# nka77/DAHiTra

Measured on AMD Instinct MI355X. Metric: image-pairs/s (256x256) train step, 1/2/4/8 MI355X + CPU ref, higher is better.
Workload: dtype bf16; 1 GPU; LEVIR-CD 256x256 synthetic pairs, base_transformer_pos_s4, bf16, batch 32 per GPU (global 32), fwd+focal+bwd+allreduce+AdamW; net_G=base_transformer_pos_s4, global_batch=32, img_size=256, parallelism=dp1, hip_graph=True, step_form=one graph (AdamW inside), attn_dtype=bf16

## Files before the change

dahitra_amd/csrc/conv_wgrad.hip:

```cpp
#include "common.h"

namespace {

constexpr int TH = 8, TW = 16;
static inline int co_tile(int Cout) { return Cout <= 16 ? 16 : (Cout <= 32 ? 32 : 64); }

struct WgArgs {
    const void* x;
    const void* dy;
    float* part;
    int N, H, W, Cin, OH, OW, Cout, pad;
    int tilesX, tilesY, splitk, groups, npix, in_npix;
    int ci_tiles;
    int CinPitch;
    int dil;
    int CoutUse;
    int direct;
    const float* in_scale;
    const float* in_shift;
    int in_groups;
    int phase_mode;
    int no_xcd_remap;
    const void* dyt_y;
    const float* dytoef;
    int dyt_groups;
    long x_split;
};

constexpr int lds_pitch(int row_bytes) { return ((row_bytes / 32) & 1) ? row_bytes : row_bytes + 32; }

union F8 {
    s16x8 v;
    s16x4 h[2];
// ... 523 lines not shown
    const int t = threadIdx.x;
    if (t < (vec ? 128 : 32)) {
        const int l2 = vec ? t >> 2 : t, e = vec ? t & 3 : 0;
        const long i2 = vec ? (block * 32 + l2) * 4 + e : block * 32 + l2;
        if (i2 < n) {
            float s = 0.f;
#pragma unroll
            for (int r = 0; r < 8; ++r) s += red[r][l2 * 4 + e];
            const int ci2 = (int)(i2 % I), o2 = (int)((i2 / I) % O), tap2 = (int)(i2 / ((long)I * O));
            const size_t d = ((size_t)o2 * I + ci2) * taps + tap2;
            if (accumulate) dw[d] += s; else dw[d] = s;
        }
    }
}
__global__ void wgrad_reduce_oihw_kernel(const float* __restrict__ part, int splitk, int taps, int Oslab, int O, int I,
                                         float* __restrict__ dw, int accumulate) {
    __shared__ float red[8][132];
    const long n = (long)O * I * taps;
    wgrad_reduce_block(part + (size_t)blockIdx.y * splitk * taps * Oslab * I, splitk, taps, Oslab, O, I,
                       dw + (size_t)blockIdx.y * n, accumulate, blockIdx.x, red);
}
struct WgReduceJob {
    const float* part;
    float* dw;
    int splitk, taps, Oslab, O, I, accumulate, first_block, nblocks;
};
__global__ void wgrad_reduce_multi_kernel(const WgReduceJob* __restrict__ jobs, int njobs) {
    __shared__ float red[8][132];
    int j = 0;
    while (j + 1 < njobs && (int)blockIdx.x >= jobs[j + 1].first_block) ++j;
    const WgReduceJob job = jobs[j];
    wgrad_reduce_block(job.part, job.splitk, job.taps, job.Oslab, job.O, job.I, job.dw, job.accumulate,
                       (long)blockIdx.x - job.first_block, red);
}

#ifdef DH_WS_TIMING
__device__ long long g_ws[4096 * 16];
#define WS_NOW() ((long long)wall_clock64())
#define WS_T(...) __VA_ARGS__
#else
#define WS_T(...)
#endif
template <int DIL>
__device__ __forceinline__ void ws_body(const WgArgs& p, int bx, int kz, const int nbx, const int nkz, unsigned char* smem) {
    constexpr int KS = 3, TAPS = 9;
    constexpr int HH = (TH - 1) + (KS - 1) * DIL + 1, HWD = (TW - 1) + (KS - 1) * DIL + 1;
    constexpr int XP = lds_pitch(128), DP = lds_pitch(128);
    constexpr int STAGE = HH * HWD * XP + TH * TW * DP;
    float* bnp = reinterpret_cast<float*>(smem + 2 * STAGE);

    const int tid = threadIdx.x, lane = tid & 63, wv = tid >> 6;
    const int pl = lane & 15, g = lane >> 4;
    if (nbx > 1 && (nkz & 7) == 0 && !p.no_xcd_remap) {
        const unsigned lin = (unsigned)(kz * nbx + bx), xcd = lin & 7, sq = lin >> 3;
        bx = (int)(sq % nbx);
        kz = (int)((sq / nbx) * 8 + xcd);
    }
    const int cot = bx / p.ci_tiles, cit = bx % p.ci_tiles;
    const int co0 = cot * 64, ci0 = cit * 64;
    const int tiles_per_img = p.tilesX * p.tilesY;
    const int ntiles = p.N * tiles_per_img;
    const int my_tiles = kz < ntiles ? (ntiles - kz + p.splitk - 1) / p.splitk : 0;

    if (p.in_scale) {
        for (int i = tid; i < p.in_groups * 128; i += 512) {
            const int gi = i >> 7, k = (i >> 6) & 1, c = i & 63;
// ... 668 lines not shown
                                     int H, int W, int Cin, int OH, int OW, int Cout, int ks, int stride, int pad,
                                     int use_tr, int Cout_real, int dilation, const float* in_scale, const float* in_shift,
                                     int in_groups, void* workspace, int* splitk_out, void* stream) {
    DH_REQUIRE(in_scale && in_shift, "conv2d_wgrad_bn_in: scale / shift missing");
    return conv2d_wgrad_impl(dtype, x, dy, dw_oihw, accumulate, N, H, W, Cin, OH, OW, Cout, ks, stride, pad, 1, 0, use_tr,
                             Cout_real, 0, dilation, workspace, stream, splitk_out ? 1 : 0, splitk_out, in_scale, in_shift,
                             in_groups);
}
extern "C" int dh_conv2d_wgrad_describe(int dtype, int accumulate, int N, int H, int W, int Cin, int OH, int OW, int Cout, int ks,
                                        int stride, int pad, int groups, int npix_valid, int use_tr, int Cout_real, int cin_pitch,
                                        int dilation, int in_groups, int has_in_scale, int split_input, int batch_open, int* out) {
    static const float on[1] = {0.f};
    DH_REQUIRE(out, "conv2d_wgrad_describe: out missing");
    return conv2d_wgrad_impl(dtype, nullptr, nullptr, nullptr, accumulate, N, H, W, Cin, OH, OW, Cout, ks, stride, pad, groups, npix_valid,
                             use_tr, Cout_real, split_input ? Cin / 2 : cin_pitch, dilation, nullptr, nullptr, 1, nullptr,
                             has_in_scale ? on : nullptr, has_in_scale ? on : nullptr, in_groups, nullptr, nullptr, 1,
                             split_input ? 16 : 0, out, batch_open, ks == 2);
}
extern "C" int dh_stem_wgrad_bn(const void* xs16, const void* d, const void* y, const float* coef, int groups, int N, int OH,
                                int OW, float* dw2, int use_tr, void* workspace, void* stream) {
    DH_REQUIRE(xs16 && d && y && coef && groups >= 1 && N % groups == 0, "stem_wgrad_bn: bad arguments (N=%d groups=%d)", N, groups);
    return conv2d_wgrad_impl(DH_DTYPE_BF16, xs16, d, dw2, 0, N, OH, OW, 16, OH, OW, 64, 4, 1, 2, 1, 0, use_tr, 0, 16, 1, workspace,
                             stream, 0, nullptr, nullptr, nullptr, 1, y, coef, groups);
}
extern "C" int dh_wgrad_reduce_job_size(void) { return (int)sizeof(WgReduceJob); }
extern "C" int dh_wgrad_reduce_outputs_per_block(int Cin) { return wgrad_reduce_epb(Cin); }
extern "C" int dh_wgrad_reduce_multi(const void* jobs_dev, int njobs, int total_blocks, void* stream) {
    if (njobs <= 0) return 0;
    hipLaunchKernelGGL(wgrad_reduce_multi_kernel, dim3(total_blocks), dim3(256), 0, reinterpret_cast<hipStream_t>(stream),
                       reinterpret_cast<const WgReduceJob*>(jobs_dev), njobs);
    DH_CHECK_LAUNCH("wgrad_reduce_multi");
    return 0;
}

extern "C" long dh_conv2d_wgrad_phase_workspace_size(int N, int H, int W, int Cin) {
    WgArgs a = wg_args(N, H, W, Cin, H, W, 32, 1);
    a.phase_mode = 1;
    WgPlan p;
    wg_plan(a, WgLaunch{WG_BF16, true, 2, 1, 0, false}, p);
    return (long)4 * p.splitk * 4 * 32 * Cin * 4;
}
extern "C" int dh_conv2d_wgrad_phase(int dtype, const void* x, const void* dy, int N, int H, int W, int Cin, int use_tr,
                                     void* workspace, int* splitk_out, void* stream) {
    DH_REQUIRE(splitk_out && workspace, "conv2d_wgrad_phase: workspace / splitk_out missing");
    DH_REQUIRE((Cin * (dtype == DH_DTYPE_BF16 ? 2 : 4)) % 16 == 0, "conv2d_wgrad_phase: Cin=%d not 16-byte aligned", Cin);
    return conv2d_wgrad_impl(dtype, x, dy, nullptr, 0, N, H, W, Cin, H, W, 32, 2, 1, 1, 1, 0, use_tr, 0, 0, 1, workspace, stream, 1,
                             splitk_out, nullptr, nullptr, 1, nullptr, nullptr, 1, 0, nullptr, 0, 1);
}

namespace {
__global__ void phase_wgrad_combine_kernel(const float* __restrict__ dwab, float* __restrict__ dw, int Cin, int accumulate) {
    const int i = blockIdx.x * blockDim.x + threadIdx.x;
    if (i >= 32 * Cin) return;
    const size_t pstride = (size_t)32 * Cin * 4;
    const float* src = dwab + (size_t)i * 4;
    float v[4][4];
#pragma unroll
    for (int ph = 0; ph < 4; ++ph) {
        const float4 q = *reinterpret_cast<const float4*>(src + ph * pstride);
        v[ph][0] = q.x; v[ph][1] = q.y; v[ph][2] = q.z; v[ph][3] = q.w;
    }
    const int ra[3][2] = {{0, 1}, {0, 1}, {0, 1}}, rt[3][2] = {{0, 0}, {1, 0}, {1, 1}};
#pragma unroll
    for (int kh = 0; kh < 3; ++kh)
#pragma unroll
        for (int kw = 0; kw < 3; ++kw) {
            float s = 0.f;
#pragma unroll
            for (int m = 0; m < 2; ++m)
#pragma unroll
                for (int n = 0; n < 2; ++n) s += v[ra[kh][m] * 2 + ra[kw][n]][rt[kh][m] * 2 + rt[kw][n]];
            float* d = dw + (size_t)i * 9 + kh * 3 + kw;
            if (accumulate) *d += s; else *d = s;
        }
}

template <typename T>
__global__ void pack_phase_weights_kernel(const float* __restrict__ w, const float* __restrict__ bias, int Cin,
                                          T* __restrict__ fwd, T* __restrict__ dgrad, float* __restrict__ bias4) {
    const int i = blockIdx.x * blockDim.x + threadIdx.x;
    if (i < 128 && bias4) bias4[i] = bias ? bias[i & 31] : 0.f;
    if (i >= 32 * Cin) return;
    const int co = i / Cin, ci = i % Cin;
    float k[3][3];
#pragma unroll
    for (int j = 0; j < 9; ++j) k[j / 3][j % 3] = w[(size_t)i * 9 + j];
    const int lo[2][2] = {{0, 1}, {0, 2}}, hi[2][2] = {{0, 2}, {1, 2}};
#pragma unroll
    for (int a = 0; a < 2; ++a)
#pragma unroll
        for (int b = 0; b < 2; ++b)
#pragma unroll
            for (int t = 0; t < 2; ++t)
#pragma unroll
                for (int u = 0; u < 2; ++u) {
                    float s = 0.f;
                    for (int kh = lo[a][t]; kh <= hi[a][t]; ++kh)
                        for (int kw = lo[b][u]; kw <= hi[b][u]; ++kw) s += k[kh][kw];
                    const int ph = a * 2 + b;
                    if (fwd) stf(fwd + ((size_t)(t * 2 + u) * 128 + ph * 32 + co) * Cin + ci, s);
                    if (dgrad) stf(dgrad + ((size_t)((1 - t) * 2 + (1 - u)) * Cin + ci) * 128 + ph * 32 + co, s);
                }
}
}

namespace {
template <typename T>
__global__ void pack_s2_dgrad_phase_kernel(const float* __restrict__ w, int Co, int Ci, T* __restrict__ out) {
    const int i = blockIdx.x * blockDim.x + threadIdx.x;
    if (i >= Co * Ci) return;
    const int co = i / Ci, ci = i % Ci;
    float k[3][3];
#pragma unroll
    for (int j = 0; j < 9; ++j) k[j / 3][j % 3] = w[(size_t)i * 9 + j];
    const int kmap[2][2] = {{-1, 1}, {2, 0}};
#pragma unroll
    for (int a = 0; a < 2; ++a)
#pragma unroll
        for (int b = 0; b < 2; ++b)
#pragma unroll
            for (int t = 0; t < 2; ++t)
#pragma unroll
                for (int u = 0; u < 2; ++u) {
                    const int kh = kmap[a][t], kw = kmap[b][u];
                    const float v = (kh >= 0 && kw >= 0) ? k[kh][kw] : 0.f;
                    stf(out + ((size_t)(t * 2 + u) * 4 * Ci + (a * 2 + b) * Ci + ci) * Co + co, v);
                }
}
}
extern "C" int dh_pack_s2_dgrad_phase_weights(int dtype, const float* w_oihw, int Co, int Ci, void* out, void* stream) {
    DH_REQUIRE((Ci == 32 || Ci == 64) && Co % 16 == 0, "pack_s2_dgrad_phase_weights: Ci=%d (32 or 64) Co=%d", Ci, Co);
    const dim3 grid(dh_cdiv(Co * Ci, 256));
    hipStream_t st = reinterpret_cast<hipStream_t>(stream);
    if (dtype == DH_DTYPE_BF16) hipLaunchKernelGGL(pack_s2_dgrad_phase_kernel<bf16>, grid, dim3(256), 0, st, w_oihw, Co, Ci, (bf16*)out);
    else hipLaunchKernelGGL(pack_s2_dgrad_phase_kernel<float>, grid, dim3(256), 0, st, w_oihw, Co, Ci, (float*)out);
    DH_CHECK_LAUNCH("pack_s2_dgrad_phase_weights");
    return 0;
}
extern "C" int dh_phase_wgrad_combine(const float* dwab, float* dw_oihw, int Cin, int accumulate, void* stream) {
    hipLaunchKernelGGL(phase_wgrad_combine_kernel, dim3(dh_cdiv(32 * Cin, 256)), dim3(256), 0, reinterpret_cast<hipStream_t>(stream),
                       dwab, dw_oihw, Cin, accumulate);
    DH_CHECK_LAUNCH("phase_wgrad_combine");
    return 0;
}
extern "C" int dh_pack_phase_weights(int dtype, const float* w_oihw, const float* bias, int Cin, void* fwd, void* dgrad,
                                     float* bias4, void* stream) {
    DH_REQUIRE(Cin % 16 == 0, "pack_phase_weights: Cin=%d", Cin);
    const dim3 grid(dh_cdiv(32 * Cin, 256));
    hipStream_t st = reinterpret_cast<hipStream_t>(stream);
    if (dtype == DH_DTYPE_BF16)
        hipLaunchKernelGGL(pack_phase_weights_kernel<bf16>, grid, dim3(256), 0, st, w_oihw, bias, Cin, (bf16*)fwd, (bf16*)dgrad, bias4);
    else
        hipLaunchKernelGGL(pack_phase_weights_kernel<float>, grid, dim3(256), 0, st, w_oihw, bias, Cin, (float*)fwd, (float*)dgrad, bias4);
    DH_CHECK_LAUNCH("pack_phase_weights");
    return 0;
}
```

dahitra_amd/csrc/loss_optim.hip:

```cpp
#include "common.h"

namespace {

constexpr int MAXC = 8;

template <int CT>
__global__ __launch_bounds__(256) void focal_kernel(const float* __restrict__ logits, const long long* __restrict__ target,
                                                    int B, int Crt, long HW, float alpha, float gscale,
                                                    float* __restrict__ dlogits, float* __restrict__ partial) {
    __shared__ float red[256];
    const int C = CT > 0 ? CT : Crt;
    constexpr int NC = CT > 0 ? CT : MAXC;
    const long total = (long)B * HW;
    float lsum = 0.f;
    const long stride = (long)gridDim.x * blockDim.x;
    const long i0 = (long)blockIdx.x * blockDim.x + threadIdx.x;
    long b = i0 / HW, p = i0 - b * HW;
    const long db = stride / HW, dp = stride - db * HW;
    for (long i = i0; i < total; i += stride) {
        float z[NC], pr[NC], lp[NC];
        float m = -INFINITY;
#pragma unroll
        for (int c = 0; c < NC; ++c)
            if (c < C) { z[c] = logits[(b * C + c) * HW + p]; m = fmaxf(m, z[c]); }
        float s = 0.f;
#pragma unroll
        for (int c = 0; c < NC; ++c)
            if (c < C) { pr[c] = expf(z[c] - m); s += pr[c]; }
        const float ls = logf(s), inv = 1.f / s;
        const int t = (int)target[i];
        float loss = 0.f, gsum = 0.f, gp[NC];
#pragma unroll
        for (int c = 0; c < NC; ++c)
            if (c < C) {
                pr[c] *= inv;
                lp[c] = z[c] - m - ls;
                const float oh = (c == t ? 1.f : 0.f) + 1e-6f;
                const float om = 1.f - pr[c];
                loss += oh * (-alpha * om * om * lp[c]);
                gp[c] = oh * (-alpha) * (-2.f * om * pr[c] * lp[c] + om * om);
                gsum += gp[c];
            }
        lsum += loss;
        if (dlogits) {
#pragma unroll
            for (int c = 0; c < NC; ++c)
                if (c < C) dlogits[(b * C + c) * HW + p] = gscale * (gp[c] - pr[c] * gsum);
        }
        b += db; p += dp;
        if (p >= HW) { p -= HW; ++b; }
    }
    red[threadIdx.x] = lsum;
    __syncthreads();
    for (int o = 128; o > 0; o >>= 1) {
        if (threadIdx.x < o) red[threadIdx.x] += red[threadIdx.x + o];
        __syncthreads();
    }
    if (threadIdx.x == 0) partial[blockIdx.x] = red[0];
}

__global__ __launch_bounds__(256) void ce_partial_kernel(const float* __restrict__ logits, const long long* __restrict__ target,
                                                         int B, int C, long HW, int ignore, double* __restrict__ partial) {
    __shared__ double sh[16];
    double ls = 0.0, cnt = 0.0;
    const long total = (long)B * HW;
    for (long i = (long)blockIdx.x * blockDim.x + threadIdx.x; i < total; i += (long)gridDim.x * blockDim.x) {
        const int t = (int)target[i];
        if (t == ignore) continue;
        const long b = i / HW, p = i % HW;
        float m = -INFINITY;
        for (int c = 0; c < C; ++c) m = fmaxf(m, logits[(b * C + c) * HW + p]);
        float s = 0.f;
        for (int c = 0; c < C; ++c) s += expf(logits[(b * C + c) * HW + p] - m);
        ls += (double)(m + logf(s) - logits[(b * C + t) * HW + p]);
        cnt += 1.0;
    }
    double r = dh_block_sum_f64(ls, sh);
    if (threadIdx.x == 0) partial[2 * blockIdx.x] = r;
    r = dh_block_sum_f64(cnt, sh);
    if (threadIdx.x == 0) partial[2 * blockIdx.x + 1] = r;
}
__global__ void ce_finalize_kernel(const double* __restrict__ partial, int nblk, float* __restrict__ out) {
    __shared__ double sh[16];
    double ls = 0.0, cnt = 0.0;
    for (int i = threadIdx.x; i < nblk; i += blockDim.x) { ls += partial[2 * i]; cnt += partial[2 * i + 1]; }
    const double a = dh_block_sum_f64(ls, sh);
    const double n = dh_block_sum_f64(cnt, sh);
    if (threadIdx.x == 0) { out[0] = (float)(a / n); out[1] = (float)n; }
}
__global__ void ce_bwd_kernel(const float* __restrict__ logits, const long long* __restrict__ target, int B, int C, long HW,
                              int ignore, const float* __restrict__ fwd_out, const float* __restrict__ upstream,
// ... 123 lines not shown
            const int c = ch % 3, r = ch / 3, ry = r >> 1, rx = r & 1;
            const int kh = 2 * (tap / 4) + ry - 1, kw = 2 * (tap % 4) + rx - 1;
            if (kh >= 0 && kh < 7 && kw >= 0 && kw < 7) v = w[((o * 3 + c) * 7 + kh) * 7 + kw] * (oscale ? oscale[o] : 1.f);
        }
        stf(out + i, v);
    }
}
__global__ void stem_unpack_grad_kernel(const float* __restrict__ dw2, float* __restrict__ dw, int O, int CP,
                                        int accumulate) {
    const int i = blockIdx.x * blockDim.x + threadIdx.x;
    if (i >= O * 147) return;
    const int kw = i % 7, kh = (i / 7) % 7, c = (i / 49) % 3, o = i / 147;
    const int dy = (kh + 1) / 2, ry = (kh + 1) % 2, dx = (kw + 1) / 2, rx = (kw + 1) % 2;
    const int ch = (ry * 2 + rx) * 3 + c;
    const float v = dw2[((long)(o * CP + ch) * 4 + dy) * 4 + dx];
    if (accumulate) dw[i] += v; else dw[i] = v;
}

}

#define ST(s) reinterpret_cast<hipStream_t>(s)
extern "C" int dh_reduce_partials(const float* partial, long nt, long n, float scale, float* out, int accumulate,
                                  void* stream);

extern "C" int dh_focal_loss(const float* logits_nchw, const long long* target, int B, int C, long HW, float alpha,
                             float grad_scale, float* loss_out, float* dlogits_nchw, void* workspace, void* stream) {
    DH_REQUIRE(C >= 1 && C <= MAXC, "focal_loss: n_class=%d unsupported (max %d)", C, MAXC);
    const long total = (long)B * HW;
    long g = (total + 255) / 256;
    if (g > 1024) g = 1024;
    float* partial = reinterpret_cast<float*>(workspace);
    auto kern = C == 2 ? focal_kernel<2> : (C == 5 ? focal_kernel<5> : focal_kernel<0>);
    hipLaunchKernelGGL(kern, dim3((int)g), dim3(256), 0, ST(stream), logits_nchw, target, B, C, HW, alpha,
                       grad_scale / (float)total, dlogits_nchw, partial);
    DH_CHECK_LAUNCH("focal_loss");
    return dh_reduce_partials(partial, g, 1, 1.0f / (float)total, loss_out, 0, stream);
}

extern "C" int dh_cross_entropy_fwd(const float* logits_nchw, const long long* target, int B, int C, long HW,
                                    int ignore_index, float* out_dev, void* workspace, void* stream) {
    DH_REQUIRE(C >= 1 && B > 0 && HW > 0, "cross_entropy: empty input");
    const long total = (long)B * HW;
    long g = (total + 255) / 256;
    if (g > 1024) g = 1024;
    double* partial = reinterpret_cast<double*>(workspace);
    hipLaunchKernelGGL(ce_partial_kernel, dim3((int)g), dim3(256), 0, ST(stream), logits_nchw, target, B, C, HW,
                       ignore_index, partial);
    hipLaunchKernelGGL(ce_finalize_kernel, dim3(1), dim3(256), 0, ST(stream), partial, (int)g, out_dev);
    DH_CHECK_LAUNCH("cross_entropy_fwd");
    return 0;
}
extern "C" int dh_cross_entropy_bwd(const float* logits_nchw, const long long* target, int B, int C, long HW,
                                    int ignore_index, const float* fwd_out_dev, const float* upstream_dev,
                                    float* dlogits_nchw, void* stream) {
    const long total = (long)B * HW;
    long g = (total + 255) / 256;
    if (g > 4096) g = 4096;
    hipLaunchKernelGGL(ce_bwd_kernel, dim3((int)g), dim3(256), 0, ST(stream), logits_nchw, target, B, C, HW, ignore_index,
                       fwd_out_dev, upstream_dev, dlogits_nchw);
    DH_CHECK_LAUNCH("cross_entropy_bwd");
    return 0;
}
extern "C" int dh_dice_argmax_constant(const float* logits_nchw, const long long* target, int B, int C, long HW, float eps,
                                       float* loss_out, void* workspace, void* stream) {
    const long total = (long)B * HW;
    long g = (total + 255) / 256;
    if (g > 1024) g = 1024;
    double* partial = reinterpret_cast<double*>(workspace);
    hipLaunchKernelGGL(dice_argmax_partial_kernel, dim3((int)g), dim3(256), 0, ST(stream), logits_nchw, target, B, C, HW,
// ... 139 lines not shown
```

dahitra_amd/csrc/pointwise.hip:

```cpp
#include "common.h"

namespace {

inline int ew_grid(long n, int block) {
    long g = (n + block - 1) / block;
    return (int)(g > 8192 ? 8192 : (g < 1 ? 1 : g));
}
#define GSL(i, n) for (long i = (long)blockIdx.x * blockDim.x + threadIdx.x; i < (n); i += (long)gridDim.x * blockDim.x)

template <typename T>
__global__ void nchw_to_nhwc_kernel(const float* __restrict__ src, T* __restrict__ dst, int N, int C, long HW, int CP) {
    const long total = (long)N * HW * CP;
    GSL(i, total) {
        const int c = (int)(i % CP);
        const long p = (i / CP) % HW;
        const long n = i / (CP * HW);
        stf(dst + i, c < C ? src[(n * C + c) * HW + p] : 0.f);
    }
}
template <typename T>
__global__ void nchw_to_nhwc_piece_kernel(const float* __restrict__ src, T* __restrict__ dst, int N, int C, long HW) {
    constexpr int V = V16<T>::N;
    const long total = (long)N * HW;
    GSL(i, total) {
        const long p = i % HW, n = i / HW;
        float v[V];
#pragma unroll
        for (int c = 0; c < V; ++c) v[c] = c < C ? src[(n * C + c) * HW + p] : 0.f;
        stv(dst + i * V, v);
    }
}
template <typename T>
__global__ void nhwc_to_nchw_kernel(const T* __restrict__ src, float* __restrict__ dst, int N, int C, long HW) {
// ... 906 lines not shown
                const int ci = (int)((i / (unsigned)j.OK) % (unsigned)j.IPad);
                const int tap = (int)(i / (unsigned)(j.OK * j.IPad));
                unsigned ok = 0;
#pragma unroll
                for (int e = 0; e < 8; ++e) ok |= (unsigned)(ci < j.I && o + e < j.O) << e;
                pack_store8(dgrad + i, j.w + (unsigned)((o * j.I + ci) * taps + (taps - 1 - tap)), (unsigned)(j.I * taps), ok);
            }
        } else {
            for (unsigned i = t0; i < (unsigned)(taps * j.IPad * j.OK); i += step) {
                const int o = (int)(i % (unsigned)j.OK);
                const int ci = (int)((i / (unsigned)j.OK) % (unsigned)j.IPad);
                const int tap = (int)(i / (unsigned)(j.OK * j.IPad));
                stf(dgrad + i, (ci < j.I && o < j.O) ? j.w[(unsigned)((o * j.I + ci) * taps + (taps - 1 - tap))] : 0.f);
            }
        }
    }
}
__global__ __launch_bounds__(256) void pack_weights_multi_kernel(const PackJob* __restrict__ jobs, int njobs) {
    int lo = 0, hi = njobs - 1;
    while (lo < hi) {
        const int mid = (lo + hi + 1) >> 1;
        if (jobs[mid].first_block <= (int)blockIdx.x) lo = mid; else hi = mid - 1;
    }
    const PackJob j = jobs[lo];
    const int lb = blockIdx.x - j.first_block;
    __shared__ __attribute__((aligned(16))) float tile[PK_T * PK_PITCH];
    if (pack_tiled(j)) {
        if ((j.dtype & 0xff) == DH_DTYPE_BF16) pack_job_tiled<bf16>(j, lb, tile); else pack_job_tiled<float>(j, lb, tile);
        return;
    }
    if ((j.dtype & 0xff) == DH_DTYPE_BF16) pack_job<bf16>(j, lb); else pack_job<float>(j, lb);
}

template <typename T>
__global__ __launch_bounds__(256) void colsum_partial_kernel(const T* __restrict__ x, long P, int C,
                                                             float* __restrict__ partial) {
    __shared__ float red[256 * 8];
    constexpr int V = sizeof(T) == 2 ? 8 : 4;
    if (C % V == 0 && C <= 1024 && 256 % (C / V) == 0) {
        const int cvn = C / V, cv = threadIdx.x % cvn, ph = threadIdx.x / cvn, nph = 256 / cvn;
        float s[4][V];
#pragma unroll
        for (int u = 0; u < 4; ++u)
#pragma unroll
            for (int j = 0; j < V; ++j) s[u][j] = 0.f;
        const long step = (long)gridDim.x * nph;
        long p = (long)blockIdx.x * nph + ph;
        auto row = [&](long r, float (&acc)[V]) {
            float v[V];
            if constexpr (V == 8) unpack16(*reinterpret_cast<const uint4*>(x + r * C + cv * V), v);
            else ld4(x + r * C + cv * V, v);
#pragma unroll
            for (int j = 0; j < V; ++j) acc[j] += v[j];
        };
        for (; p + 3 * step < P; p += 4 * step) {
            row(p, s[0]); row(p + step, s[1]); row(p + 2 * step, s[2]); row(p + 3 * step, s[3]);
        }
        for (int u = 0; p < P; p += step, ++u) row(p, s[u & 3]);
        float* mine = red + threadIdx.x * V;
#pragma unroll
        for (int j = 0; j < V; ++j) mine[j] = (s[0][j] + s[1][j]) + (s[2][j] + s[3][j]);
        __syncthreads();
        for (int c = threadIdx.x; c < C; c += 256) {
            float t = 0.f;
            for (int r = 0; r < nph; ++r) t += red[(r * cvn + c / V) * V + (c % V)];
            partial[(long)blockIdx.x * C + c] = t;
// ... 263 lines not shown
}
extern "C" int dh_absdiff_bwd(int dtype, const void* a, const void* b, const void* dy, void* da, void* db, long n, int accumulate, void* stream) {
    if (dtype == DH_DTYPE_BF16) hipLaunchKernelGGL(absdiff_bwd_kernel<bf16>, dim3(ew_grid(n, 256)), dim3(256), 0, ST(stream), (const bf16*)a, (const bf16*)b, (const bf16*)dy, (bf16*)da, (bf16*)db, n, accumulate);
    else hipLaunchKernelGGL(absdiff_bwd_kernel<float>, dim3(ew_grid(n, 256)), dim3(256), 0, ST(stream), (const float*)a, (const float*)b, (const float*)dy, (float*)da, (float*)db, n, accumulate);
    DH_CHECK_LAUNCH("absdiff_bwd");
    return 0;
}
extern "C" int dh_zero_insert2(int dtype, const void* dy, void* z, int N, int OH, int OW, int H, int W, int C, void* stream) {
    DH_REQUIRE(C % 4 == 0, "zero_insert2: C %% 4");
    const long n = (long)N * H * W * (C / 4);
    if (dtype == DH_DTYPE_BF16) hipLaunchKernelGGL(zero_insert2_kernel<bf16>, dim3(ew_grid(n, 256)), dim3(256), 0, ST(stream), (const bf16*)dy, (bf16*)z, N, OH, OW, H, W, C);
    else hipLaunchKernelGGL(zero_insert2_kernel<float>, dim3(ew_grid(n, 256)), dim3(256), 0, ST(stream), (const float*)dy, (float*)z, N, OH, OW, H, W, C);
    DH_CHECK_LAUNCH("zero_insert2");
    return 0;
}
extern "C" int dh_add_coarse(int dtype, void* x, const void* coarse, int N, int OH, int OW, int H, int W, int C, void* stream) {
    const int V = dtype == DH_DTYPE_BF16 ? 8 : 4;
    DH_REQUIRE(C % V == 0 && x && coarse && OH == (H + 1) / 2 && OW == (W + 1) / 2, "add_coarse: C=%d, %dx%d <- %dx%d", C, H, W, OH, OW);
    const long n = (long)N * OH * OW * (C / V);
    if (dtype == DH_DTYPE_BF16) hipLaunchKernelGGL(add_coarse_kernel<bf16>, dim3(ew_grid(n, 256)), dim3(256), 0, ST(stream), (bf16*)x, (const bf16*)coarse, N, OH, OW, H, W, C);
    else hipLaunchKernelGGL(add_coarse_kernel<float>, dim3(ew_grid(n, 256)), dim3(256), 0, ST(stream), (float*)x, (const float*)coarse, N, OH, OW, H, W, C);
    DH_CHECK_LAUNCH("add_coarse");
    return 0;
}
extern "C" int dh_pack_weight(int dtype, const float* w_oihw, const float* out_scale, int O, int I, int ks, int OPad, void* fwd, int IPad, int dgrad_inner, void* dgrad, void* stream) {
    const int OK = dgrad_inner > O ? dgrad_inner : O;
    const long n = (long)ks * ks * (OPad > IPad ? OPad : IPad) * (OK > I ? OK : I);
    if (dtype == DH_DTYPE_BF16) hipLaunchKernelGGL(pack_weight_kernel<bf16>, dim3(ew_grid(n, 256)), dim3(256), 0, ST(stream), w_oihw, out_scale, O, I, ks, OPad, (bf16*)fwd, IPad, OK, (bf16*)dgrad);
    else hipLaunchKernelGGL(pack_weight_kernel<float>, dim3(ew_grid(n, 256)), dim3(256), 0, ST(stream), w_oihw, out_scale, O, I, ks, OPad, (float*)fwd, IPad, OK, (float*)dgrad);
    DH_CHECK_LAUNCH("pack_weight");
    return 0;
}
extern "C" int dh_pack_job_size(void) { return (int)sizeof(PackJob); }
extern "C" int dh_pack_weights_multi(const void* jobs_dev, int njobs, int total_blocks, void* stream) {
    if (njobs <= 0) return 0;
    hipLaunchKernelGGL(pack_weights_multi_kernel, dim3(total_blocks), dim3(256), 0, ST(stream),
                       reinterpret_cast<const PackJob*>(jobs_dev), njobs);
    DH_CHECK_LAUNCH("pack_weights_multi");
    return 0;
}
extern "C" int dh_colsum(int dtype, const void* x, long P, int C, float* out, int accumulate, void* workspace, void* stream) {
    DH_REQUIRE(C >= 1 && C <= 256, "colsum: C=%d out of range", C);
    const long rows_per_pass = 256 / (C >= 4 && (C & 3) == 0 ? C / 4 : C);
    long want = (P + rows_per_pass * 8 - 1) / (rows_per_pass * 8);
    const int grid = (int)(want < 64 ? 64 : (want > 256 ? 256 : want));
    float* partial = reinterpret_cast<float*>(workspace);
    if (dtype == DH_DTYPE_BF16) hipLaunchKernelGGL(colsum_partial_kernel<bf16>, dim3(grid), dim3(256), 0, ST(stream), (const bf16*)x, P, C, partial);
    else hipLaunchKernelGGL(colsum_partial_kernel<float>, dim3(grid), dim3(256), 0, ST(stream), (const float*)x, P, C, partial);
    DH_CHECK_LAUNCH("colsum");
    return dh_reduce_partials(partial, grid, C, 1.0f, out, accumulate, stream);
}
extern "C" int dh_cast_from_f32(int dtype, const float* src, void* dst, long n, void* stream) {
    if (dtype == DH_DTYPE_BF16) hipLaunchKernelGGL(cast_from_f32_kernel<bf16>, dim3(ew_grid(n, 256)), dim3(256), 0, ST(stream), src, (bf16*)dst, n);
    else hipLaunchKernelGGL(cast_from_f32_kernel<float>, dim3(ew_grid(n, 256)), dim3(256), 0, ST(stream), src, (float*)dst, n);
    DH_CHECK_LAUNCH("cast_from_f32");
    return 0;
}
extern "C" int dh_cast_to_f32(int dtype, const void* src, float* dst, long n, int accumulate, void* stream) {
    if (dtype == DH_DTYPE_BF16) hipLaunchKernelGGL(cast_to_f32_kernel<bf16>, dim3(ew_grid(n, 256)), dim3(256), 0, ST(stream), (const bf16*)src, dst, n, accumulate);
    else hipLaunchKernelGGL(cast_to_f32_kernel<float>, dim3(ew_grid(n, 256)), dim3(256), 0, ST(stream), (const float*)src, dst, n, accumulate);
    DH_CHECK_LAUNCH("cast_to_f32");
    return 0;
}

namespace {
template <typename T>
__device__ __forceinline__ void absdiff_halves_body(const T* __restrict__ tok, T* __restrict__ out, int B, long n, int bid, int nb) {
    GSLB(i, (long)B * n, bid, nb) {
        const long b = i / n, j = i % n;
        stf(out + i, fabsf(ldf(tok + (b * 2 + 1) * n + j) - ldf(tok + (b * 2) * n + j)));
    }
}
template <typename T>
__global__ void absdiff_halves_kernel(const T* __restrict__ tok, T* __restrict__ out, int B, long n) {
    absdiff_halves_body<T>(tok, out, B, n, blockIdx.x, gridDim.x);
}
template <typename T>
__device__ __forceinline__ void absdiff_halves_bwd_body(const T* __restrict__ tok, const T* __restrict__ dout, T* __restrict__ dtok,
                                                        int B, long n, int bid, int nb) {
    GSLB(i, (long)B * n, bid, nb) {
        const long b = i / n, j = i % n;
        const float df = ldf(tok + (b * 2 + 1) * n + j) - ldf(tok + (b * 2) * n + j);
        const float g = (df > 0.f ? 1.f : (df < 0.f ? -1.f : 0.f)) * ldf(dout + i);
// ... 92 lines not shown
```

dahitra_amd/engine.py:

```python
import os
import sys
import types

import torch

from . import ops
from .netspec import (ATTN_SCALE, BIT_DIM_HEAD, BIT_HEADS, BN_EPS, BN_MOMENTUM, DIM, LN_EPS, UNET_LEVELS,
                      get_config, is_active, state_spec)

RELU, GELU, NONE = ops.ACT_RELU, ops.ACT_GELU, ops.ACT_NONE



def _drain(gen):
    try:
        while True:
            next(gen)
    except StopIteration as e:
        return e.value


class Packed:
    __slots__ = ("fwd", "dgrad", "fwd_frag", "dgrad_frag")

# ... 38 lines not shown
        self.fused_bn_bwd = os.environ.get("DAHITRA_BN_FUSION", "0") == "1"
        self.coarse_shortcut = os.environ.get("DAHITRA_NO_COARSE_SHORTCUT", "0") != "1"
        self.lazy_bn = os.environ.get("DAHITRA_NO_LAZY_BN", "0") != "1"
        self.phase_conv_pred = os.environ.get("DAHITRA_NO_PHASE_CONV", "0") != "1"
        self.phase_s2_dgrad = os.environ.get("DAHITRA_NO_PHASE_S2", "0") != "1"
        self.phase_up_conv = os.environ.get("DAHITRA_NO_PHASE_UPCONV", "0") != "1"
        self.split_cat = os.environ.get("DAHITRA_NO_SPLIT_CAT", "0") != "1"
        self.direct_stem = os.environ.get("DAHITRA_NO_DIRECT_STEM", "0") != "1"
        self.fused_stem_bwd = os.environ.get("DAHITRA_NO_FUSED_STEM_BWD", "0") != "1"
        self.fused_head_out = os.environ.get("DAHITRA_NO_FUSED_HEAD", "0") != "1"
        self.defer_dec_finalize = os.environ.get("DAHITRA_NO_DEFER_DEC_FINALIZE", "0") != "1"
        self.fuse_dec_stack = os.environ.get("DAHITRA_NO_DEC_STACK", "0") != "1"
        self.level_streams = os.environ.get("DAHITRA_LEVEL_STREAMS", "0") == "1"
        self._lstreams = []
        self.gated_head_dgrad = os.environ.get("DAHITRA_GATED_HEAD", "0") == "1"
        self.fused_head_bn = os.environ.get("DAHITRA_NO_FUSED_HEAD_BN", "0") != "1"
        self.fused_up4_bwd = os.environ.get("DAHITRA_NO_FUSED_UP4_BWD", "0") != "1"
        self.fused_up4_fwd = os.environ.get("DAHITRA_FUSED_UP4_FWD", "0") == "1"
        self.use_side = os.environ.get("DAHITRA_SIDE_STREAM", "0") == "1"
        self.pack_side = os.environ.get("DAHITRA_PACK_SIDE", "0") == "1"
        self._pack_stream = None
        self.side = None
        self._deferred_wgrad = None
        self.shapes = {k: s for k, s, _ in state_spec(net_G)}
        self.p = {}
        self.g = {}
        self.pk = {}
        self.wstack = {}
        self.training = False
        self.need_grad = False
        self._bwd = None
        self._plans = {}
        self._wgrad_plan = None

    def bind(self, params, grads):
        self.p, self.g = params, grads
        self._plans = {}

    def _pack_all(self):
        plan = self._plans.get(self.need_grad)
        if plan is None:
            plan = self._plans[self.need_grad] = self._build_plan()
        pack, self.pk, self.xstack, self.wstack = plan
        if self.pack_side and self.training and self.direct_stem and self.dtype == torch.bfloat16 and ops.PROFILE is None:
            if self._pack_stream is None:
                self._pack_stream = ops.SideStream(self.p["resnet.conv1.weight"].device)
            with self._pack_stream.fork():
                pack.run()
        else:
            pack.run()
        key = "resnet.conv1.weight"
        if not (self.direct_stem and self.dtype == torch.bfloat16):
            self.pk[key] = Packed(ops.stem_pack_weight(self.p[key], self.dtype), None)

    def _pack_join(self):
        if self._pack_stream is not None:
            self._pack_stream.join()

    def _build_plan(self):
        ck = ops.chunk_channels(self.dtype)
        pack = ops.PackPlan(self.p["resnet.conv1.weight"].device)
        pk, xstack = {}, {}
        wstack = {}
        for key, shape in self.shapes.items():
            if key not in self.p or not key.endswith("weight") or len(shape) not in (2, 4):
                continue
            if not is_active(self.net_G, key) or key == "resnet.conv1.weight":
                continue
            if key.startswith("conv_a") or key.startswith("conv_token") or key.startswith("resnet.fc") or \
                    key.startswith("resnet.layer4"):
                continue
            if key == "conv_pred.weight" and self.phase_conv_pred and shape[1] % 64 == 0 and self.cfg["kind"] == "bit":
                continue
            if self.phase_up_conv and key in ("conv_layer2.0.weight", "conv_layer3.0.weight", "conv_layer4.0.weight") and \
                    tuple(shape[:2]) == (32, 32):
                continue
            if ".to_q." in key or ".to_k." in key or ".to_v." in key or \
                    (".to_out." in key and "transformer_decoder" in key):
                pfx, rest = key.split(".layers.")
                li, which = int(rest.split(".")[0]), rest.split(".fn.fn.")[1]
                skey = (pfx, which)
                if skey not in xstack:
                    depth = 1 + max(int(k.split(".layers.")[1].split(".")[0]) for k in self.shapes
                                    if k.startswith(pfx + ".layers.") and k.endswith(which))
                    xstack[skey] = torch.empty(depth, shape[0] * shape[1], dtype=self.dtype, device=self.p[key].device)
                view = xstack[skey][li]
                pack.add(self.p[key], self.dtype, want_fwd=False, out_dgrad=view)
                pk[key] = Packed(None, view)
                continue
            O = shape[0]
            dt = self.dtype
            if key.startswith("transformer_decoder") and ".1.fn.fn.net." in key and len(shape) == 2 and shape[0] % 16 == 0 and \
                    shape[1] % 16 == 0:
                pfx, rest = key.split(".layers.")
                li, which = int(rest.split(".")[0]), ("net.0" if ".net.0." in key else "net.3")
                if (pfx, which) not in wstack:
                    depth = 1 + max(int(k.split(".layers.")[1].split(".")[0]) for k in self.shapes
                                    if k.startswith(pfx + ".layers.") and k.endswith("1.fn.fn.%s.weight" % which))
                    mk = lambda: torch.empty(depth, shape[0] * shape[1], dtype=dt, device=self.p[key].device)
                    wstack[(pfx, which)] = (mk(), mk() if self.need_grad else None)
                sf, sd = wstack[(pfx, which)]
                f, d = pack.add(self.p[key], dt, want_dgrad=self.need_grad, dgrad_inner=O, out_fwd=sf[li].view(1, shape[0], shape[1]),
                                out_dgrad=sd[li].view(1, shape[1], shape[0]) if sd is not None else None)
                pk[key] = Packed(f, d)
                continue
            if key.startswith("transformer") and not key.startswith("transformer_decoder"):
                dt = torch.float32
            c = ops.chunk_channels(dt)
            f, d = pack.add(self.p[key], dt, want_dgrad=self.need_grad, dgrad_inner=-(-O // c) * c)
            ff = dd = None
            if dt == torch.bfloat16 and len(shape) == 4 and shape[2] == 3 and \
                    ((O in (64, 128, 256) and shape[1] in (64, 128, 256)) or (O == 32 and shape[1] == 32)):
                ff, dd = pack.add(self.p[key], dt, want_dgrad=self.need_grad, dgrad_inner=O, frag=True)
            pk[key] = Packed(f, d, ff, dd)
        return pack, pk, xstack, wstack

    def s2_phase_ok(self, ks, stride, pad, xshape, dy):
        N, H, W, Cin = xshape
        return self.phase_s2_dgrad and ks == 3 and stride == 2 and pad == 1 and Cin in (32, 64) and \
            H == 2 * dy.shape[1] and W == 2 * dy.shape[2] and dy.shape[-1] % ops.chunk_channels(self.dtype) == 0

    def conv_dgrad(self, dy, wkey, ks, stride, pad, xshape, residual=None, dilation=1, gate=None, coarse=False):
        N, H, W, Cin = xshape
        flops = 2.0 * dy.shape[0] * dy.shape[1] * dy.shape[2] * self.shapes[wkey][0] * Cin * ks * ks
        if coarse:
            assert ks == 1 and stride == 2 and residual is None and gate is None
            return ops.conv2d(dy, self.pk[wkey].dgrad, Cin, 1, 1, 0, alg_flops=flops)
        if gate is None and self.s2_phase_ok(ks, stride, pad, xshape, dy):
            wph = ops.pack_s2_dgrad_phase_weights(self.p[wkey], self.dtype)
            if residual is None or isinstance(residual, CoarseRes):
                return ops.conv3x3s2_dgrad(dy, wph, Cin, residual.t if residual is not None else None, alg_flops=flops)
            return ops.add(ops.conv3x3s2_dgrad(dy, wph, Cin, None, alg_flops=flops), residual)
        assert not isinstance(residual, CoarseRes)
        if stride == 2:
            dy = ops.zero_insert2(dy, H, W)
        r = ops.conv2d(dy, self.pk[wkey].dgrad, Cin, ks, 1, dilation * (ks - 1) - pad, residual=residual,
                       out_hw=(H, W), alg_flops=flops, dilation=dilation, gate=gate,
                       w_frag=self.pk[wkey].dgrad_frag if stride == 1 else None)
        return Gated(*r) if gate is not None else r

    def conv_bn(self, x, wkey, bnkey, ks, stride, pad, groups, relu, residual=None, dilation=1, lazy=False, side_wgrad=False):
        cout = self.shapes[wkey][0]
        lazy = lazy and self.training and self.lazy_bn and relu and residual is None and not self.fused_bn_bwd
        gamma, beta = self.p[bnkey + ".weight"], self.p[bnkey + ".bias"]
        rm, rv = self.p[bnkey + ".running_mean"], self.p[bnkey + ".running_var"]
        act = RELU if relu else NONE
        split = isinstance(x, ops.SplitCat)
        if split and not (self.training and ks == 3 and stride == 1 and pad == 1 and dilation == 1 and residual is None):
            x, split = x.materialize(), False
        relu_bits = None
        if self.training:
            if split:
                y, st = ops.conv3x3_split(x, self.pk[wkey].fwd, self.pk[wkey].fwd_frag, cout, want_stats=True)
            else:
                y, st = ops.conv2d(x, self.pk[wkey].fwd, cout, ks, stride, pad, want_stats=True, dilation=dilation,
                                   w_frag=self.pk[wkey].fwd_frag if stride == 1 else None)
            N, OH, OW, _ = y.shape
            mean, invstd, scale, shift = ops.bn_finalize(st, cout, groups, (N // groups) * OH * OW, gamma, beta, rm, rv,
                                                         BN_MOMENTUM, BN_EPS, nbt=self.p[bnkey + ".num_batches_tracked"])
            if lazy:
                out = ops.BnInput(y, scale, shift, groups)
            elif relu and residual is not None and self.need_grad:
# ... 25 lines not shown
            else:
                r = ops.bn_bwd(dout, out if relu else None, y, mean, invstd, gamma, self.g[bnkey + ".weight"],
                               self.g[bnkey + ".bias"], groups, accumulate=True, want_dres=has_res, bits=relu_bits)
                dy, dres = r if has_res else (r, None)
            if side_wgrad and self.side is not None:
                self._deferred_wgrad = (x, dy, wkey, ks, stride, pad, dilation)
            else:
                ops.conv2d_wgrad(x, dy, self.g[wkey], ks, stride, pad, accumulate=True, use_tr=self.use_tr,
                                 dilation=dilation)
            if through_up4 is not None:
                return ops.conv3x3_dgrad_through_up4(dy, self.pk[wkey].dgrad, *through_up4), dres
            if split and need_dx:
                assert dx_res is None and next_gate is None and not coarse_dx
                cin = x.shape[-1]
                return ops.conv3x3_split(dy, self.pk[wkey].dgrad, self.pk[wkey].dgrad_frag, cin, split_out=True,
                                         alg_flops=2.0 * dy.shape[0] * dy.shape[1] * dy.shape[2] * cout * cin * 9), dres
            dx = self.conv_dgrad(dy, wkey, ks, stride, pad, x.shape, residual=dx_res, dilation=dilation,
                                 gate=next_gate, coarse=coarse_dx) if need_dx else None
            return dx, dres
        bwd.gate = (out if relu else None, y, mean, invstd, groups) if (self.fused_bn_bwd and cout % 16 == 0) else None
        bwd.bn = (y, scale, shift, mean, invstd, groups) if (self.training and relu and not has_res) else None
        return out, bwd

    def conv_act(self, x, wkey, bkey, ks, pad, act, cpad_grad=False):
        cout = self.shapes[wkey][0]
        out = ops.conv2d(x, self.pk[wkey].fwd, cout, ks, 1, pad, bias=self.p[bkey] if bkey else None, act=act)
        if not self.need_grad:
            return out, None

        def bwd(dout, need_dx=True, dx_res=None, masked=False):
            dy = ops.act_bwd(dout, out, RELU) if (act == RELU and not masked) else dout
            ops.conv2d_wgrad(x, dy, self.g[wkey], ks, 1, pad, accumulate=True, use_tr=self.use_tr)
            if bkey:
                ops.colsum(dy.view(-1, cout), self.g[bkey], accumulate=True)
            dx = self.conv_dgrad(dy, wkey, ks, 1, pad, x.shape, residual=dx_res) if need_dx else None
            return dx
        return out, bwd

    def conv_pred_phase(self, x):
        wkey, bkey = "conv_pred.weight", "conv_pred.bias"
        wf, wd, b4 = ops.pack_phase_weights(self.p[wkey], self.p[bkey], self.dtype)
        out = ops.conv_up2_fwd(x, wf, b4)
        if not self.need_grad:
            return out, None

        def bwd(dout):
            ops.conv_up2_wgrad(x, dout, self.g[wkey], accumulate=True, use_tr=self.use_tr)
            ops.colsum(dout.view(-1, 32), self.g[bkey], accumulate=True)
            return ops.conv_up2_dgrad(dout, wd, x.shape[-1])
        return out, bwd

    def stem(self, x1, x2, groups, pool=False):
        B = x1.shape[0]
        H, W = x1.shape[2], x1.shape[3]
        wkey, bnkey = "resnet.conv1.weight", "resnet.bn1"
        gamma, beta = self.p[bnkey + ".weight"], self.p[bnkey + ".bias"]
        rm, rv = self.p[bnkey + ".running_mean"], self.p[bnkey + ".running_var"]
        oh, ow = H // 2, W // 2
        direct = self.direct_stem and self.dtype == torch.bfloat16
        if not direct:
            cp = ops.chunk_channels(self.dtype)
            xs = torch.empty(2 * B, H // 2, W // 2, cp, dtype=self.dtype, device=x1.device)
            ops.stem_space_to_depth_into(x1, xs[:B])
            ops.stem_space_to_depth_into(x2, xs[B:])
        if self.training:
            if direct:
                y, st, xs = ops.stem7_fwd(x1, x2, self.p[wkey], want_stats=True, want_xs=self.need_grad, groups=groups)
            else:
                y, st = ops.conv2d(xs, self.pk[wkey].fwd, 64, 4, 1, 2, want_stats=True, out_hw=(oh, ow))
            mean, invstd, scale, shift = ops.bn_finalize(st, 64, groups, B * oh * ow, gamma, beta, rm, rv, BN_MOMENTUM,
                                                         BN_EPS, nbt=self.p[bnkey + ".num_batches_tracked"])
            if pool:
                out = None
                pooled, parg = ops.maxpool(y, want_arg=True, bn=(scale, shift, groups))
            else:
                out = ops.bn_apply(y, scale, shift, groups, RELU)
        else:
            scale, shift = ops.bn_eval_params(gamma, beta, rm, rv, BN_EPS)
            if direct:
                out = ops.stem7_fwd(x1, x2, self.p[wkey], out_scale=scale, bias=shift, relu=True)[0]
            else:
# ... 398 lines not shown
        xn, st1 = ops.layernorm(x0, g1, b1, LN_EPS)
        wqT, wkT, wvT = (self.pk[a + ".fn.to_%s.weight" % n].dgrad for n in "qkv")
        woT = self.pk[a + ".fn.to_out.0.weight"].dgrad
        prep = ops.XattnPrep(tok, tok_b, tok_s, B, images, L, heads, dim_head, g1, b1, wq, wkT, wvT, woT, self.dtype,
                             ATTN_SCALE, LN_EPS)
        HLP = prep.HLP
        dots = ops.linear(xn, prep.kq, HLP, images=images, w_image_stride=HLP * DIM)
        attn = ops.softmax_groups(dots, heads, L)
        x1 = ops.linear(attn, prep.voT, DIM, bias=bo, residual=x0, images=images, w_image_stride=HLP * DIM)
        if not self.need_grad:
            return x1, None
        dev = x0.device

        def bwd(dx1):
            dattn = ops.linear(dx1, prep.vo, HLP, images=images, w_image_stride=HLP * DIM)
            dvoT = torch.empty(images, DIM, HLP, dtype=torch.float32, device=dev)
            ops.linear_wgrad(attn, dx1, dvoT, images=images, per_image=True, use_tr=self.use_tr)
            ops.colsum(dx1, self.g[a + ".fn.to_out.0.bias"], accumulate=True)
            ddots = ops.softmax_groups_bwd(attn, dattn, heads, L)
            dxn = ops.linear(ddots, prep.kqT, DIM, images=images, w_image_stride=HLP * DIM)
            dkq = torch.empty(images, HLP, DIM, dtype=torch.float32, device=dev)
            ops.linear_wgrad(xn, ddots, dkq, images=images, per_image=True, use_tr=self.use_tr)
            dx = ops.layernorm_bwd(dxn, x0, st1, g1, self.g[a + ".norm.weight"], self.g[a + ".norm.bias"],
                                   dx_add=dx1, accumulate=True)
            ops.xattn_prep_bwd(prep, tok, dtok, g1, wqT, wk, wv, wo, dkq, dvoT, self.g[a + ".norm.weight"],
                               self.g[a + ".norm.bias"], *(self.g[a + ".fn.to_%s.weight" % n] for n in "qkv"),
                               self.g[a + ".fn.to_out.0.weight"], True, self.dtype)
            return dx
        return x1, bwd

    def forward(self, x1, x2, training, need_grad):
        ops.set_f32_mma_mode(self.mma_fwd)
        self.training, self.need_grad = training, need_grad
        if need_grad and self.use_side and self.side is None and self.dtype == torch.bfloat16:
            self.side = ops.SideStream(x1.device)
        self._pack_all()
        if self.cfg["kind"] == "bit":
            logits, bwd = self._bit(x1, x2)
        else:
            logits, bwd = self._unet(x1, x2)
        if need_grad:
            self._bwd = bwd
        if self.mma_fwd == 3 and not self._x3_checked and not torch.cuda.is_current_stream_capturing():
            self._x3_checked = True
            if not bool(torch.isfinite(logits).all()):
                raise FloatingPointError(
                    "dahitra_amd: compute_dtype='bf16x3' produced non-finite logits in its fp16-plane forward (operands beyond "
                    "fp16's range: |x| < 65504, |w| < 255); set DAHITRA_X3_FWD=2 (three bf16 planes, six products, fp32's range)")
        return logits

    def split_prefixes(self):
        if self.cfg["kind"] == "bit":
            return ("resnet.conv1.", "resnet.bn1.", "resnet.layer1.", "resnet.layer2.")
        return ("resnet.",)

    def take_backward(self):
        bwd, self._bwd = self._bwd, None
        return bwd

    def backward(self, dlogits_nchw, bwd=None):
        ops.set_f32_mma_mode(self.mma_bwd)
        if bwd is None:
            bwd, self._bwd = self._bwd, None
        if bwd is None:
            raise RuntimeError("dahitra_amd: backward called without a grad-enabled forward")
        plan = self._plans.get(True)
# ... 31 lines not shown
            return
        x, dy, wkey, ks, stride, pad, dilation = d
        with self.side.fork(x.y if isinstance(x, ops.BnInput) else (x.a if isinstance(x, ops.Up4Input) else x), dy):
            ops.conv2d_wgrad(x, dy, self.g[wkey], ks, stride, pad, accumulate=True, use_tr=self.use_tr, dilation=dilation)

    def _side_join(self):
        if self.side is not None:
            self.run_deferred_wgrad()
            self.side.join()

    def backward_second(self):
        ops.set_f32_mma_mode(self.mma_bwd)
        second, state = self._split_state
        self._split_state = None
        try:
            second(state)
            self._wgrad_plan.run()
        finally:
            self._wgrad_plan.__exit__(*sys.exc_info())

    def _head_out(self, h, wkey, bkey):
        ncls = self.shapes[wkey][0]
        ck = ops.chunk_channels(self.dtype)
        if self.pk[wkey].fwd.shape[-2] == 16 and self.fused_head_out:
            out = ops.conv3x3_head(h, self.pk[wkey].fwd, ncls, self.p[bkey], w_oihw=self.p[wkey])
        else:
            out = ops.nhwc_to_nchw(ops.conv2d(h, self.pk[wkey].fwd, ncls, 3, 1, 1, bias=self.p[bkey]))
        if not self.need_grad:
            return out, None

        small = 8 if (self.dtype == torch.bfloat16 or ncls > 4) else 4
        direct = h.shape[-1] == 32 and ncls <= small

        def bwd(dl_nchw, next_gate=None, head_bn=None, relu_out=None):
            if direct and next_gate is None:
                fuse = self.fused_head_bn and ncls <= 8 and self.g[wkey].is_contiguous() and \
                    (self.dtype == torch.bfloat16 or (self.dtype == torch.float32 and ops.get_f32_mma_mode() != 0))
                if head_bn is not None and fuse:
                    return HeadGrad(ops.head_dlogits_pack(dl_nchw, self.dtype), self.p[wkey], ncls, self.g[wkey], self.g[bkey])
                if relu_out is not None and fuse and relu_out is h:
                    return ops.head_relu_bwd(ops.head_dlogits_pack(dl_nchw, self.dtype), self.p[wkey], ncls, h, self.g[wkey],
                                             self.g[bkey])
                dl = ops.nchw_to_nhwc(dl_nchw, self.dtype, cpad=small)
                ops.conv2d_wgrad(h, dl, self.g[wkey], 3, 1, 1, accumulate=True, use_tr=self.use_tr, cout_real=ncls)
                tmp = torch.empty(small, dtype=torch.float32, device=h.device)
                ops.colsum(dl.view(-1, small), tmp)
                ops.reduce_rows(tmp, 1, ncls, self.g[bkey], accumulate=True)
                if head_bn is not None and self.gated_head_dgrad and self.dtype == torch.bfloat16 and ncls <= 2:
                    return Gated(*ops.head_dgrad3x3_bn(dl, self.p[wkey], ncls, *head_bn))
                return ops.head_dgrad3x3(dl, self.p[wkey], ncls, relu_out=relu_out)
            dl = ops.nchw_to_nhwc(dl_nchw, self.dtype, cpad=ck)
            ops.conv2d_wgrad(h, dl, self.g[wkey], 3, 1, 1, accumulate=True, use_tr=self.use_tr, cout_real=ncls)
            tmp = torch.empty(ck, dtype=torch.float32, device=h.device)
            ops.colsum(dl.view(-1, ck), tmp)
            ops.reduce_rows(tmp, 1, ncls, self.g[bkey], accumulate=True)
            dh = self.conv_dgrad(dl, wkey, 3, 1, 1, h.shape, gate=next_gate)
            return ops.act_bwd(dh, relu_out, RELU) if relu_out is not None else dh
        return out, bwd

    def _bit(self, x1, x2):
        cfg, L = self.cfg, self.cfg["token_len"]
        B = x1.shape[0]
        S2 = 2 * B
        xp, xarg, xshape, b_stem = self.stem(x1, x2, 2, pool=True)
        self._pack_join()
        if cfg.get("backbone") == "resnet50":
            l1, b_l1 = self.res50_layer(xp, 1, 1, 1, 1, 2)
            l2, b_l2 = self.res50_layer(l1, 2, 2, 1, 1, 2)
            l3, b_l3 = self.res50_layer(l2, 3, 1, 1, 2, 2)
        else:
            l1, b_l1 = self.res_layer(xp, 1, 1, 2)
            l2, b_l2 = self.res_layer(l1, 2, 2, 2)
            l3, b_l3 = self.res_layer(l2, 3, 1, 2)
        phased = self.phase_conv_pred and l3.shape[-1] % 64 == 0
        if phased:
            feat, b_pred = self.conv_pred_phase(l3)
        else:
            up = ops.upsample2(l3)
            feat, b_pred = self.conv_act(up, "conv_pred.weight", "conv_pred.bias", 3, 1, NONE)
        _, fh, fw, _ = feat.shape
        hw = fh * fw
        wa = self.p["conv_a.weight"]
        tok_cat, tsaved = ops.tokenizer_fwd(feat, wa, self.p["pos_embedding"], B, L)
        tok2d, b_enc = self.encoder(tok_cat.view(B * 2 * L, DIM), "transformer", cfg["enc_depth"], BIT_HEADS,
                                    BIT_DIM_HEAD, B, 2 * L)
        dtok = torch.zeros_like(tok2d) if self.need_grad else None
        dec, b_dec = self.decoder(feat.view(S2 * hw, DIM), S2, tok2d, 2 * L * DIM, L * DIM, B, dtok,
                                  "transformer_decoder", cfg["dec_depth"], BIT_HEADS, cfg["dec_dim_head"], L)
        dec4 = dec.view(S2, fh, fw, DIM)
        k0 = "classifier.0.weight"
        if self.fused_up4_fwd and self.dtype == torch.bfloat16 and DIM == 32 and tuple(self.shapes[k0][:2]) == (32, 32) and \
                tuple(self.pk[k0].fwd.shape) == (9, 32, 32):
            upd = ops.Up4Input(dec4[:B].contiguous(), dec4[B:].contiguous())
        else:
            upd = ops.absdiff_upsample4(dec4[:B], dec4[B:])
        h, b_c0 = self.conv_bn(upd, k0, "classifier.1", 3, 1, 1, 1, True, lazy=True, side_wgrad=True)
        logits, b_out = self._head_out(h, "classifier.3.weight", "classifier.3.bias")
        if not self.need_grad:
            return logits, None

        def bwd_first(dl):
            dh = b_out(dl, next_gate=b_c0.gate, head_bn=getattr(b_c0, "bn", None))
            fuse = self.fused_up4_bwd and self.dtype == torch.bfloat16 and fh % 2 == 0 and fw % 4 == 0 and \
                self.pk["classifier.0.weight"].dgrad.dim() == 3 and self.pk["classifier.0.weight"].dgrad.shape[1] == 32
            if fuse:
                dec_g = torch.empty_like(dec4)
                b_c0(dh, through_up4=(dec4[:B], dec4[B:], dec_g[:B], dec_g[B:]))
            else:
                dupd, _ = b_c0(dh)
                dec_g = torch.empty_like(dec4)
                ops.absdiff_upsample4_bwd_into(dec4[:B], dec4[B:], dupd, dec_g[:B], dec_g[B:])
            dfeat = b_dec(dec_g.view(S2 * hw, DIM))
            if self.side is not None:
                self.run_deferred_wgrad()
            dtok_cat = b_enc(dtok)
            dfeat4 = dfeat.view(S2, fh, fw, DIM)
            ops.tokenizer_bwd(feat, wa, tsaved, dtok_cat, dfeat4, self.g["conv_a.weight"], self.g["pos_embedding"],
                              B, L, accumulate=True)
            dl3 = b_pred(dfeat4) if phased else ops.upsample2_bwd(b_pred(dfeat4))
            return b_l3(dl3, next_gate=b_l2.gate)

        def bwd_second(dl2):
            dxp = b_l1(b_l2(dl2, next_gate=b_l1.gate))
            if hasattr(b_stem, "from_pool"):
                b_stem.from_pool(xarg, dxp)
            else:
                b_stem(ops.maxpool_bwd(xarg, dxp, xshape))

        def bwd(dl):
            bwd_second(bwd_first(dl))
        bwd.split = (bwd_first, bwd_second, ("resnet.conv1.", "resnet.bn1.", "resnet.layer1.", "resnet.layer2."))
        return logits, bwd
# ... 105 lines not shown
        pos = self.p["pos_embedding_decoder_3"] if (with_pos and self.cfg["decoder_pos"]) else None
        xin = ops.add_pos(dxc, pos) if pos is not None else dxc
        out, b_dec = yield from self._decoder_gen(xin.view(B * hw, DIM), B, dtk.view(B * L, DIM), L * DIM, 0, B, ddtk,
                                                  "transformer_decoder_%d" % l, lv["dec_depth"], lv["heads"], lv["dim_head"], L)
        out4 = out.view(B, fh, fw, DIM)
        if not self.need_grad:
            return out4, None

        def bwd(dout4):
            dxin = (yield from b_dec(dout4.reshape(B * hw, DIM))).view(B, fh, fw, DIM)
            if pos is not None:
                ops.add_pos_bwd(dxin, self.g["pos_embedding_decoder_3"], accumulate=True)
            dcat = b_cdec(dxin)
            dtok = torch.zeros_like(tok2d)
            ops.absdiff_halves_bwd(tk3, ddtk, dtok)
            dtok_cat = b_enc(dtok)
            yield
            dsq = ops.split_halves(dcat)
            gpos = self.g["pos_embedding_3"] if with_pos else torch.zeros(1, 2 * L, DIM, device=sq.device)
            ops.tokenizer_bwd(sq, wa, tsaved, dtok_cat, dsq, self.g["conv_token_%d.weight" % l], gpos, B, L,
                              accumulate=True)
            yield
            return b_sq(dsq)
        return out4, bwd

    def _up_conv(self, l, x):
        wkey, bkey = "conv_layer%d.0.weight" % l, "conv_layer%d.0.bias" % l
        if not (self.phase_up_conv and x.shape[-1] == 32 and self.shapes[wkey][0] == 32):
            up = ops.upsample2(x)
            out, b = self.conv_act(up, wkey, bkey, 3, 1, RELU)
            if not self.need_grad:
                return out, None
            return out, (lambda d, masked=False: ops.upsample2_bwd(b(d, masked=masked)))
        wf, wd, b4 = ops.pack_phase_weights(self.p[wkey], self.p[bkey], self.dtype)
        out = ops.conv_up2_fwd(x, wf, b4, act=RELU)
        if not self.need_grad:
            return out, None

        def bwd(dout, masked=False):
            dy = dout if masked else ops.act_bwd(dout, out, RELU)
            ops.conv_up2_wgrad(x, dy, self.g[wkey], accumulate=True, use_tr=self.use_tr)
            ops.colsum(dy.view(-1, 32), self.g[bkey], accumulate=True)
            return ops.conv_up2_dgrad(dy, wd, 32)
        return out, bwd

    def _unet(self, x1, x2):
        B = x1.shape[0]
        s2, b_stem = self.stem(x1, x2, 2)
        self._pack_join()
        p4, arg4 = ops.maxpool(s2, want_arg=True)
        s4, b_l1 = self.res_layer(p4, 1, 1, 2)
        s8, b_l2 = self.res_layer(s4, 2, 2, 2)
        p16, arg16 = ops.maxpool(s8, want_arg=True)
        s16, b_l3 = self.res_layer(p16, 3, 1, 2)
        level = self._xbd_level if self.cfg["kind"] == "xbd" else self._level
        if self.need_grad:
            self._zpool = [torch.zeros(3 * 3 * B * self.cfg["token_len"] * DIM, dtype=torch.float32, device=s4.device), 0]
        ew = self.cfg["kind"] != "xbd"
        (o5, b5), (t4, b4), (t3, b3) = self._run_staged([level(5, s16, B), level(4, s8, B), level(3, s4, B)], ew=ew)
        self._zpool = None
        o5u = ops.upsample2(o5)
        o4, bu4 = self._up_conv(4, ops.add(t4, o5u))
        o3, bu3 = self._up_conv(3, ops.add(t3, o4))
        _, h2, w2, c2 = s2.shape
        k20 = "conv_layer2_0.0.weight"
        split2 = self.split_cat and self.training and self.pk[k20].fwd_frag is not None and \
            (not self.need_grad or self.pk[k20].dgrad_frag is not None) and \
            ops.conv3x3_split_supported(B, h2, w2, 2 * c2, self.shapes[k20][0], self.dtype)
        cat2 = ops.SplitCat(s2) if split2 else ops.SplitCat(s2).materialize()
        y, b20 = self.conv_bn(cat2, k20, "conv_layer2_0.1", 3, 1, 1, 1, True, lazy=True)
        y2 = ops.conv2d(y, self.pk["conv_layer2_0.3.weight"].fwd, 32, 3, 1, 1, bias=self.p["conv_layer2_0.3.bias"],
                        residual=o3)
        o2, bu2 = self._up_conv(2, y2)
        logits, b_out = self._head_out(o2, "classifier.weight", "classifier.bias")
        if not self.need_grad:
            return logits, None

        def bwd_first(dl):
            do2 = b_out(dl, relu_out=o2)
            dy2 = bu2(do2, masked=True)
            ops.conv2d_wgrad(y, dy2, self.g["conv_layer2_0.3.weight"], 3, 1, 1, accumulate=True, use_tr=self.use_tr)
            ops.colsum(dy2.view(-1, 32), self.g["conv_layer2_0.3.bias"], accumulate=True)
            dy = self.conv_dgrad(dy2, "conv_layer2_0.3.weight", 3, 1, 1, y.shape, gate=b20.gate)
            dcat2, _ = b20(dy)
            if split2:
                ds2 = dcat2
            else:
                ds2 = ops.split_halves(dcat2)
            dsum3 = bu3(dy2)
            dsum4 = bu4(dsum3)
            ds4, ds8, ds16 = self._run_staged([b3(dsum3), b4(dsum4), b5(ops.upsample2_bwd(dsum4))], ew=ew)
            return ds16, ds8, ds4, ds2

        def bwd_second(state):
            ds16, ds8, ds4, ds2 = state
            dp16 = b_l3(ds16)
            ds8 = ops.add(ds8, ops.maxpool_bwd(arg16, dp16, s8.shape))
            ds4 = ops.add(ds4, b_l2(ds8))
            dp4 = b_l1(ds4)
            if hasattr(b_stem, "from_pool") and os.environ.get("DAHITRA_NO_FUSED_STEM_BWD_UNET", "0") != "1":
                b_stem.from_pool(arg4, dp4, extra=ds2)
            else:
                b_stem(ops.add(ds2, ops.maxpool_bwd(arg4, dp4, s2.shape)))

        def bwd(dl):
            bwd_second(bwd_first(dl))
        bwd.split = (bwd_first, bwd_second, ("resnet.",))
        return logits, bwd
```

dahitra_amd/graph.py:

```python
import os

import torch
import torch.distributed as dist

from . import ops, parallel
from .models import losses


class GraphedTrainStep:
    CHECK_EVERY = 64

    def __init__(self, net, opt, a, b, lab, warmup=3, confusion=None):
        if not getattr(opt, "capturable", False):
            raise ValueError("GraphedTrainStep needs dahitra_amd.optim.AdamW(..., capturable=True)")
        self.net, self.opt = net, opt
        self.confusion = confusion
        self.world = dist.get_world_size() if dist.is_initialized() else 1
        self.exchange = parallel.exchange_enabled()
        self.split_off = None
        self.persist_bn_launches = None
        self._set_inputs(a, b, lab)
        net._ensure_arena(a.device)
        flat0 = net._arena.flat.clone()
        bufs0 = [t.clone() for t in net.buffers()]
# ... 36 lines not shown
        else:
            self.split_off = None
            with torch.cuda.graph(self.graph, stream=cs):
                self.loss = self._body(include_opt=not self.exchange)
        self._pinned = ops.pin_captured_buffers(net)
        self._generation = net._arena.generation
        self._calls = 0
        torch.cuda.synchronize()
        ops.bn_persist_check(a.device)

    def _set_inputs(self, a, b, lab):
        self.a, self.b, self.lab = a.clone(), b.clone(), lab.clone()

    def _copy_inputs(self, a, b, lab):
        self.a.copy_(a, non_blocking=True)
        self.b.copy_(b, non_blocking=True)
        self.lab.copy_(lab, non_blocking=True)

    def _eager_body(self, include_opt):
        logits = self.net(self.a, self.b)
        self.logits = logits.detach()
        self.opt.zero_grad()
        loss = losses.focal_loss(logits, self.lab)
        loss.backward()
        self._count(self.logits)
        if include_opt:
            self.opt.step()
        return loss.detach()

    def _body(self, include_opt):
        if type(self)._eager_body is not GraphedTrainStep._eager_body or os.environ.get("DAHITRA_GRAPH_AUTOGRAD") == "1":
            return self._eager_body(include_opt)
        net = self.net
        logits = self._forward_split()
        bwd = net._engine.take_backward()
        self.logits = logits
        loss, dl = self._loss_and_grad(logits)
        self._count(logits)
        net._arena.grad.zero_()
        net._engine.backward(dl, bwd)
        net._bind_grad_views()
        if include_opt:
            self.opt.step()
        return loss

    def _forward_split(self):
        return self.net._run_forward(self.a, self.b, need_grad=True)

    def _loss_and_grad(self, logits):
        tgt = self.lab[:, 0] if self.lab.dim() == logits.dim() else self.lab
        return ops.focal_loss(logits, tgt.to(torch.int64).contiguous(), want_grad=True)

    def _count(self, logits):
        if self.confusion is not None:
            tgt = self.lab[:, 0] if self.lab.dim() == logits.dim() else self.lab
            ops.confusion_matrix(logits, tgt.to(torch.int64).contiguous(), self.confusion)

    def _can_split(self):
        self.split_off = parallel.split_offset(self.net, self.world)
        return self.split_off is not None

    def _split_first(self):
        net = self.net
        logits = self._forward_split()
        bwd = net._engine.take_backward()
        self.logits = logits
        loss, dl = self._loss_and_grad(logits)
        self._count(logits)
        net._arena.grad.zero_()
        net._engine.backward_first(dl, bwd)
        net._bind_grad_views()
        return loss

    def _second(self):
        if os.environ.get("DAHITRA_OVERLAP_PERSIST_BN") == "1":
            self.net._engine.backward_second()
            return
        with ops.no_persist_bn():
            self.net._engine.backward_second()

    def _after_replay(self):
        parallel.allreduce_net_grads_(self.net)
        self._update()

    def _replay_overlapped(self):
        _, grad = self.net.flat_params()
        self.graph.replay()
        w1 = dist.all_reduce(grad[self.split_off:], op=dist.ReduceOp.SUM, async_op=True)
        self.graph2.replay()
        w2 = dist.all_reduce(grad[:self.split_off], op=dist.ReduceOp.SUM, async_op=True)
        w1.wait()
        w2.wait()
        self._update()

    def _update(self):
        self.opt.step()

    def __call__(self, *inputs):
        if self.net._arena.generation != self._generation:
            raise RuntimeError("dahitra_amd: the net's parameter arena was rebuilt (moved to another device / "
                               "parameters replaced) after this step was captured; build a new GraphedTrainStep")
        if inputs and inputs[0] is not None:
# ... 246 lines not shown
```

dahitra_amd/ops.py:

```python
import bisect
import ctypes
import math
import os
import sys

import torch

from . import _lib

ACT_NONE, ACT_RELU, ACT_GELU = 0, 1, 2
_DT = {torch.float32: 0, torch.bfloat16: 1}
_vp = ctypes.c_void_p


def dt(t):
    try:
        return _DT[t.dtype]
    except KeyError:
        raise TypeError("dahitra_amd: unsupported activation dtype %s" % t.dtype)


def set_f32_mma_mode(mode):
    _lib.check(_lib.lib().dh_set_f32_mma_mode(int(mode)), "dh_set_f32_mma_mode")

# ... 31 lines not shown
def S():
    return _vp(torch.cuda.current_stream().cuda_stream)


_ws = {}


def workspace(nbytes, device):
    key = (str(device), torch.cuda.current_stream(device).cuda_stream) if torch.device(device).type == "cuda" else str(device)
    buf = _ws.get(key)
    if buf is None or buf.numel() < nbytes:
        buf = torch.empty(max(int(nbytes), 1 << 20), dtype=torch.uint8, device=device)
        _ws[key] = buf
    return buf


def rekey_workspace(device, old_stream, new_stream):
    buf = _ws.pop((str(device), old_stream.cuda_stream), None)
    if buf is not None:
        cur = _ws.get((str(device), new_stream.cuda_stream))
        if cur is None or cur.numel() < buf.numel():
            _ws[(str(device), new_stream.cuda_stream)] = buf


_PINNED = []


def pin_captured_buffers(net):
    keep = list(_ws.values())
    eng = net._engine
    if eng._wgrad_plan is not None:
        keep += list(eng._wgrad_plan.slots) + list(eng._wgrad_plan.tables.values())
    for pack, _, xstack, wstack in eng._plans.values():
        keep += [pack.table] + list(pack.keep) + list(xstack.values())
        for fwd_stack, dgrad_stack in wstack.values():
            keep += [fwd_stack, dgrad_stack]
    keep += [net._arena.flat, net._arena.grad]
    keep = [t for t in keep if t is not None]
    _PINNED.extend(keep)
    return keep


def _call(name, *args):
    L = _lib.lib()
    _lib.check(getattr(L, name)(*args), name)


def cdiv(a, b):
    return (a + b - 1) // b


def pad16(c):
    return cdiv(c, 16) * 16


def pack_weight(w, dtype, want_dgrad=True, dgrad_inner=0, out_scale=None, want_fwd=True, out_dgrad=None):
    if w.dim() == 2:
        O, I = w.shape
        ks = 1
    else:
        O, I, ks, _ = w.shape
    OPad, IPad = pad16(O), pad16(I)
    OK = max(O, dgrad_inner)
    fwd = torch.empty(ks * ks, OPad, I, dtype=dtype, device=w.device) if want_fwd else None
    if out_dgrad is not None:
        assert out_dgrad.numel() == ks * ks * IPad * OK and out_dgrad.dtype == dtype
        dg = out_dgrad
    else:
        dg = torch.empty(ks * ks, IPad, OK, dtype=dtype, device=w.device) if want_dgrad else None
    _call("dh_pack_weight", _DT[dtype], P(w), P(out_scale), O, I, ks, OPad, P(fwd), IPad, OK, P(dg), S())
    return fwd, dg


class PackPlan:

    class _Job(ctypes.Structure):
        _fields_ = [("w", ctypes.c_void_p), ("fwd", ctypes.c_void_p), ("dgrad", ctypes.c_void_p), ("O", ctypes.c_int),
                    ("I", ctypes.c_int), ("KS", ctypes.c_int), ("OPad", ctypes.c_int), ("IPad", ctypes.c_int),
                    ("OK", ctypes.c_int), ("dtype", ctypes.c_int), ("first_block", ctypes.c_int), ("nblocks", ctypes.c_int)]

    def __init__(self, device):
        self.device, self.jobs, self.blocks, self.table, self.keep = device, [], 0, None, []

    def add(self, w, dtype, want_fwd=True, want_dgrad=True, dgrad_inner=0, out_dgrad=None, frag=False, out_fwd=None):
        if w.dim() == 2:
            (O, I), ks = w.shape, 1
        else:
            O, I, ks, _ = w.shape
        OPad, IPad, OK = pad16(O), pad16(I), max(O, dgrad_inner)
        ck = chunk_channels(dtype)
        if frag:
            assert ks == 3 and dtype == torch.bfloat16 and I % 32 == 0 and OK % 32 == 0 and out_dgrad is None
            fwd = torch.empty(OPad // 16, I // 32, ks * ks, 64, 8, dtype=dtype, device=w.device) if want_fwd else None
            dg = torch.empty(IPad // 16, OK // 32, ks * ks, 64, 8, dtype=dtype, device=w.device) if want_dgrad else None
        else:
            fwd = out_fwd if out_fwd is not None else \
                (torch.empty(ks * ks, OPad, I, dtype=dtype, device=w.device) if want_fwd else None)
            dg = out_dgrad if out_dgrad is not None else \
                (torch.empty(ks * ks, IPad, OK, dtype=dtype, device=w.device) if want_dgrad else None)
        n = max(fwd.numel() if fwd is not None else 0, dg.numel() if dg is not None else 0)
        assert n < 2 ** 31 and w.numel() < 2 ** 31, "pack_weights_multi indexes a layer with 32-bit arithmetic"
        nb = max(1, min(256, cdiv(n, 2048)))
        if ks == 3 and O % 32 == 0 and I % 32 == 0 and OK == O:
            nb = min(256, (O // 32) * (I // 32))
        self.jobs.append(self._Job(w.data_ptr(), fwd.data_ptr() if fwd is not None else None,
                                   dg.data_ptr() if dg is not None else None, O, I, ks, OPad, IPad, OK,
                                   _DT[dtype] | (0x200 if frag else 0), self.blocks, nb))
        self.blocks += nb
        self.keep += [w, fwd, dg]
        return fwd, dg

    def run(self):
        if not self.jobs:
            return
        if self.table is None:
            assert ctypes.sizeof(self._Job) == _lib.lib().dh_pack_job_size()
            raw = b"".join(bytes(j) for j in self.jobs)
            self.table = torch.frombuffer(bytearray(raw), dtype=torch.uint8).to(self.device)
        _call("dh_pack_weights_multi", P(self.table), len(self.jobs), self.blocks, S())


class WgradPlan:

    class _Job(ctypes.Structure):
        _fields_ = [("part", ctypes.c_void_p), ("dw", ctypes.c_void_p), ("splitk", ctypes.c_int), ("taps", ctypes.c_int),
                    ("Oslab", ctypes.c_int), ("O", ctypes.c_int), ("I", ctypes.c_int), ("accumulate", ctypes.c_int),
                    ("first_block", ctypes.c_int), ("nblocks", ctypes.c_int)]

    def __init__(self, device, batch=False):
        self.device, self.slots, self.cur, self.blocks = device, [], 0, 0
        self.tables, self.sigs, self.phase = {}, {}, 0
        self._prev = None
        self.post = []
        self.batch = batch and os.environ.get("DAHITRA_WGRAD_BATCH", "1") != "0"
        self.batching, self.keep = False, []

    def __enter__(self):
        global _WGRAD_PLAN
        self._prev, _WGRAD_PLAN = _WGRAD_PLAN, self
        self.cur = 0
        self.jobs = []
        self.post = []
        self.blocks = 0
        self.phase = 0
        self.keep = []
        self.batching = self.batch and PROFILE is None
        if self.batching:
            _call("dh_wgrad_batch_begin")
        elif self._prev is None:
            _call("dh_wgrad_batch_abort")
        return self

    def __exit__(self, *exc):
        global _WGRAD_PLAN
        _WGRAD_PLAN = self._prev
        if self.batching:
            self.batching = False
            if exc and exc[0] is not None:
                _lib.lib().dh_wgrad_batch_abort()
            else:
                _call("dh_wgrad_batch_end", S())
            self.keep = []
        return False

    def hold(self, *tensors):
        if self.batching:
            self.keep += [t for t in tensors if t is not None]

    def slab(self, nbytes):
        if self.cur == len(self.slots):
            self.slots.append(torch.empty(max(int(nbytes), 16), dtype=torch.uint8, device=self.device))
        elif self.slots[self.cur].numel() < nbytes:
            _PINNED.append(self.slots[self.cur])
            self.slots[self.cur] = torch.empty(int(nbytes), dtype=torch.uint8, device=self.device)
            self.tables = {}
        buf = self.slots[self.cur]
        self.cur += 1
        return buf

    def add(self, part, dw, splitk, taps, oslab, o, i, accumulate):
        nb = cdiv(o * i * taps, _lib.lib().dh_wgrad_reduce_outputs_per_block(i))
        self.jobs.append(self._Job(part.data_ptr(), dw.data_ptr(), splitk, taps, oslab, o, i, int(accumulate),
                                   self.blocks, nb))
        self.blocks += nb

    def run(self):
        if self.batching:
            _call("dh_wgrad_batch_launch", S())
            self.keep = []
        if self.jobs:
            self._run_reduce()
        for fn in self.post:
            fn()
        self.jobs, self.post, self.blocks = [], [], 0
        self.phase += 1

    def _run_reduce(self):
        sig = b"".join(bytes(j) for j in self.jobs)
        if self.tables.get(self.phase) is None or sig != self.sigs.get(self.phase):
            if torch.cuda.is_current_stream_capturing():
                raise RuntimeError("dahitra_amd: the weight-gradient plan changed during graph capture; run one eager "
                                   "step of the same shapes first")
            assert ctypes.sizeof(self._Job) == _lib.lib().dh_wgrad_reduce_job_size()
            if self.tables.get(self.phase) is not None:
                _PINNED.append(self.tables[self.phase])
            self.tables[self.phase] = torch.frombuffer(bytearray(sig), dtype=torch.uint8).to(self.device)
            self.sigs[self.phase] = sig
        _call("dh_wgrad_reduce_multi", P(self.tables[self.phase]), len(self.jobs), self.blocks, S())


_WGRAD_PLAN = None


class SideStream:

    def __init__(self, device):
        self.stream, self.keep, self.active, self._ctx = torch.cuda.Stream(device=device), [], False, None

    def fork(self, *tensors):
        global _PERSIST_BLOCK
        self.stream.wait_stream(torch.cuda.current_stream())
        self.keep += [t for t in tensors if t is not None]
        if not self.active:
            _PERSIST_BLOCK += 1
        self.active = True
        return self

    def __enter__(self):
        self._ctx = torch.cuda.stream(self.stream)
        self._ctx.__enter__()
        return self

    def __exit__(self, *exc):
        self._ctx.__exit__(*exc)
        self._ctx = None
        return False

    def join(self):
        global _PERSIST_BLOCK
        if self.active:
            torch.cuda.current_stream().wait_stream(self.stream)
# ... 285 lines not shown
    plan = _WGRAD_PLAN if defer else None
    ws = plan.slab(nbytes) if plan is not None else workspace(nbytes, x.device)
    sk = (ctypes.c_int * 1)()
    with _Prof("conv_wgrad<%s,ks%d,s%d>" % ("bf16" if x.dtype == torch.bfloat16 else "f32", ks, stride),
               2.0 * N * OH * OW * Cout * Cin * ks * ks, _nb(x, dy)):
        _call("dh_conv2d_wgrad_bn_in", dt(x), P(x), P(dy), P(dw), accumulate, N, H, W, Cin, OH, OW, Cout, ks, stride, pad, use_tr,
              cout_real, dilation, P(b.scale), P(b.shift), b.groups, P(ws), sk if plan is not None else None, S())
    if plan is not None:
        plan.hold(x, dy, b.scale, b.shift)
    if plan is not None and sk[0] > 0:
        plan.add(ws, dw, sk[0], ks * ks, Cout, cout_real if cout_real else Cout, Cin, accumulate)


def pack_phase_weights(w, bias, dtype):
    O, I = w.shape[0], w.shape[1]
    assert O == 32 and tuple(w.shape[2:]) == (3, 3)
    fwd = torch.empty(4, 128, I, dtype=dtype, device=w.device)
    dg = torch.empty(4, I, 128, dtype=dtype, device=w.device)
    b4 = torch.empty(128, dtype=torch.float32, device=w.device)
    _call("dh_pack_phase_weights", _DT[dtype], P(w), P(bias), I, P(fwd), P(dg), P(b4), S())
    return fwd, dg, b4


def conv_up2_fwd(x, wfwd, bias4, act=ACT_NONE):
    N, H, W, Cin = x.shape
    y = torch.empty(N, 2 * H, 2 * W, 32, dtype=x.dtype, device=x.device)
    key = "conv_phase<%s,up2_fwd>" % ("bf16" if x.dtype == torch.bfloat16 else "f32")
    with _Prof(key, 2.0 * N * 4 * H * W * 32 * Cin * 9, _nb(x, y, wfwd)):
        _call("dh_conv2d_fwd", dt(x), P(x), P(wfwd), P(y), P(bias4), _vp(0), _vp(0), N, H, W, Cin, H, W, 128, 128, 2, 1, 1, act,
              0, 0, _vp(0), 1, *_gate_args(None), *_bn_in_args(None), 1, _vp(0), S())
    return y


def pack_s2_dgrad_phase_weights(w, dtype):
    Co, Ci = w.shape[0], w.shape[1]
    out = torch.empty(4, 4 * Ci, Co, dtype=dtype, device=w.device)
    _call("dh_pack_s2_dgrad_phase_weights", _DT[dtype], P(w), Co, Ci, P(out), S())
    return out


def conv3x3s2_dgrad(dy, wphase, cin, coarse_residual=None, alg_flops=0):
    N, OH, OW, Co = dy.shape
    dx = torch.empty(N, 2 * OH, 2 * OW, cin, dtype=dy.dtype, device=dy.device)
    key = "conv_phase<%s,s2_dgrad>" % ("bf16" if dy.dtype == torch.bfloat16 else "f32")
    with _Prof(key, alg_flops if alg_flops else 2.0 * N * OH * OW * Co * cin * 9, _nb(dy, dx, wphase, coarse_residual)):
        _call("dh_conv2d_fwd", dt(dy), P(dy), P(wphase), P(dx), _vp(0), P(coarse_residual), _vp(0), N, OH, OW, Co, OH, OW,
              4 * cin, 4 * cin, 2, 1, 1, ACT_NONE, 0, 0, _vp(0), 1, *_gate_args(None), *_bn_in_args(None), 1, _vp(0), S())
    return dx


def conv_up2_dgrad(dy, wdgrad, cin):
    N, H2, W2, C = dy.shape
    assert C == 32 and H2 % 2 == 0 and W2 % 2 == 0 and (cin % 64 == 0 or cin == 32)
    H, W = H2 // 2, W2 // 2
    dx = torch.empty(N, H, W, cin, dtype=dy.dtype, device=dy.device)
    key = "conv_phase<%s,up2_dgrad>" % ("bf16" if dy.dtype == torch.bfloat16 else "f32")
    with _Prof(key, 2.0 * N * H2 * W2 * 32 * cin * 9, _nb(dy, dx, wdgrad)):
        _call("dh_conv2d_fwd", dt(dy), P(dy), P(wdgrad), P(dx), _vp(0), _vp(0), _vp(0), N, H, W, 128, H, W, cin, cin, 2, 1, 1,
              ACT_NONE, 0, 0, _vp(0), 1, *_gate_args(None), *_bn_in_args(None), 2, _vp(0), S())
    return dx


def conv_up2_wgrad(x, dy, dw, accumulate=True, use_tr=True):
    N, H, W, Cin = x.shape
    L = _lib.lib()
    plan, own = _WGRAD_PLAN, False
    if plan is None:
        plan, own = WgradPlan(x.device), True
        plan.__enter__()
    try:
        ws = plan.slab(L.dh_conv2d_wgrad_phase_workspace_size(N, H, W, Cin))
        dwab = plan.slab(4 * 32 * Cin * 4 * 4).view(torch.float32)
        sk = (ctypes.c_int * 1)()
        with _Prof("conv_wgrad<%s,ks3,s1>" % ("bf16" if x.dtype == torch.bfloat16 else "f32"),
                   2.0 * N * 4 * H * W * 32 * Cin * 9, _nb(x, dy)):
            _call("dh_conv2d_wgrad_phase", dt(x), P(x), P(dy), N, H, W, Cin, use_tr, P(ws), sk, S())
        per = sk[0] * 4 * 32 * Cin * 4
        for ph in range(4):
            plan.add(ws[ph * per:], dwab[ph * 32 * Cin * 4:], sk[0], 4, 32, 32, Cin, False)
        plan.post.append(lambda: _call("dh_phase_wgrad_combine", P(dwab), P(dw), Cin, accumulate, S()))
        if own:
            plan.run()
    finally:
        if own:
            plan.__exit__()


def linear_wgrad(x2d, dy2d, dw, accumulate=False, images=1, per_image=False, use_tr=True):
    rows, Cin = x2d.shape
    Cout = dy2d.shape[1]
    rpi = rows // images
    Hh = cdiv(rpi, 16)
    groups = images if per_image else 1
    L = _lib.lib()
    nbytes = L.dh_conv2d_wgrad_workspace_size(images, Hh, 16, Cin, Cout, 1, groups)
    ws = workspace(nbytes, x2d.device)
    assert images == 1 or rpi % 16 == 0
    _call("dh_conv2d_wgrad", dt(x2d), P(x2d), P(dy2d), P(dw), accumulate, images, Hh, 16, Cin, Hh, 16, Cout, 1, 1, 0, groups, rpi,
          use_tr, 0, 0, 1, P(ws), S())


def add_coarse_(x, coarse):
    N, H, W, C = x.shape
    n2, OH, OW, c2 = coarse.shape
    assert n2 == N and c2 == C and x.dtype == coarse.dtype and x.is_contiguous() and coarse.is_contiguous()
    _call("dh_add_coarse", dt(x), P(x), P(coarse), N, OH, OW, H, W, C, S())
    return x


def zero_insert2(dy, H, W):
    N, OH, OW, C = dy.shape
    z = torch.empty(N, H, W, C, dtype=dy.dtype, device=dy.device)
    _call("dh_zero_insert2", dt(dy), P(dy), P(z), N, OH, OW, H, W, C, S())
# ... 21 lines not shown
    B, C, H, W = x1.shape
    assert C == 3 and x1.dtype == torch.float32 and x1.is_contiguous() and (x2 is None or (x2.shape == x1.shape and x2.is_contiguous()))
    N = B if x2 is None else 2 * B
    y = torch.empty(N, H // 2, W // 2, 64, dtype=torch.bfloat16, device=x1.device)
    nt = _lib.lib().dh_stem7_fwd_num_slots(N, H, W, groups)
    stats = torch.empty(2, 64, nt, dtype=torch.float32, device=x1.device) if want_stats else None
    xs = torch.empty(N, H // 2, W // 2, 16, dtype=torch.bfloat16, device=x1.device) if want_xs else None
    with _Prof("stem7_fwd", 2.0 * N * (H // 2) * (W // 2) * 64 * 147, _nb(x1, x2, y, xs)):
        _call("dh_stem7_fwd", P(x1), P(x2), B, N, H, W, P(w), P(out_scale), P(bias), relu, P(y), P(stats), groups, P(xs), S())
    return y, stats, xs


def stem_pool_bn_bwd(arg, dpool, y, scale, shift, mean, invstd, gamma, dgamma, dbeta, groups, accumulate=True, extra=None):
    N, H, W, C = y.shape
    d = torch.empty_like(y)
    coef = torch.empty(groups, 3, C, dtype=torch.float32, device=y.device)
    L = _lib.lib()
    ws = workspace(L.dh_stem_pool_bn_bwd_workspace_size(C, groups), y.device)
    assert extra is None or (extra.shape == y.shape and extra.dtype == y.dtype)
    with _Prof("bn_bwd", 0, _nb(arg, dpool, y, d, extra)):
        _call("dh_stem_pool_bn_bwd_plus", P(arg), P(dpool), P(extra), P(y), P(scale), P(shift), P(mean), P(invstd), P(gamma), N,
              H, W, C, groups, P(d), P(coef), P(dgamma), P(dbeta), accumulate, P(ws), S())
    return d, coef


def stem_wgrad(x_s2d, dy, dw, accumulate=False, use_tr=True, bn=None):
    N, H2, W2, cp = x_s2d.shape
    O = dy.shape[-1]
    dw2 = torch.empty(O, 16, 4, 4, dtype=torch.float32, device=dy.device)
    if bn is not None:
        y, coef, groups = bn
        assert cp == 16 and O == 64 and y.shape == dy.shape
        L = _lib.lib()
        ws = workspace(L.dh_conv2d_wgrad_workspace_size(N, H2, W2, 16, O, 4, 1), dy.device)
        with _Prof("conv_wgrad<bf16,ks4,s1>", 2.0 * N * H2 * W2 * O * 16 * 16, _nb(x_s2d, dy, y)):
            _call("dh_stem_wgrad_bn", P(x_s2d), P(dy), P(y), P(coef), groups, N, H2, W2, P(dw2), use_tr, P(ws), S())
    else:
        conv2d_wgrad(x_s2d, dy, dw2, ks=4, stride=1, pad=2, use_tr=use_tr, cin=16, defer=False)
    _call("dh_stem_unpack_grad", P(dw2), P(dw), O, 16, accumulate, S())


def bn_finalize(stats, C, groups, count, gamma, beta, running_mean, running_var, momentum=0.1, eps=1e-5, nbt=None):
    _, cp, nt = stats.shape
    dev = stats.device
    mean = torch.empty(groups, C, dtype=torch.float32, device=dev)
    invstd, scale, shift = torch.empty_like(mean), torch.empty_like(mean), torch.empty_like(mean)
    _call("dh_bn_finalize", P(stats), nt, cp, C, groups, float(count), P(gamma), P(beta), P(running_mean), P(running_var),
          momentum, eps, P(mean), P(invstd), P(scale), P(shift), P(nbt), S())
    return mean, invstd, scale, shift


def bn_eval_params(gamma, beta, rm, rv, eps=1e-5):
    C = gamma.numel()
    scale = torch.empty(1, C, dtype=torch.float32, device=gamma.device)
    shift = torch.empty_like(scale)
    _call("dh_bn_eval_params", P(gamma), P(beta), P(rm), P(rv), eps, C, P(scale), P(shift), S())
    return scale, shift


RELU_BITS = os.environ.get("DAHITRA_NO_RELU_BITS", "0") != "1"


def bn_apply(x, scale, shift, groups=1, act=ACT_NONE, residual=None, want_bits=False):
    C = x.shape[-1]
    npix = x.numel() // C
    y = torch.empty_like(x)
    bits = None
    v = 8 if x.dtype == torch.bfloat16 else 4
    if want_bits and RELU_BITS and act == ACT_RELU and C % v == 0:
# ... 315 lines not shown
    return y


def absdiff_upsample4_bwd(a, b, dy):
    N, H, W, C = a.shape
    da, db = torch.empty_like(a), torch.empty_like(b)
    _call("dh_absdiff_upsample4_bwd", dt(a), P(a), P(b), P(dy), P(da), P(db), N, H, W, C, S())
    return da, db


def conv3x3_dgrad_through_up4(dy, wdgrad, a, b, da=None, db=None):
    N, H, W, C = a.shape
    assert C == 32 and a.dtype == torch.bfloat16 and dy.shape[:3] == (N, 4 * H, 4 * W) and wdgrad.shape[-2] == 32
    L = _lib.lib()
    partial = torch.empty(L.dh_conv3x3_dgrad_up4_partial_floats(N, 4 * H, 4 * W), dtype=torch.float32, device=a.device)
    with _Prof("conv_mfma<bf16,ks3,s1,nt32>", 2.0 * N * 16 * H * W * 32 * dy.shape[-1] * 9, _nb(dy, wdgrad, partial)):
        _call("dh_conv3x3_dgrad_up4", dt(dy), P(dy), P(wdgrad), N, 4 * H, 4 * W, dy.shape[-1], P(partial), S())
    da = torch.empty_like(a) if da is None else da
    db = torch.empty_like(b) if db is None else db
    _call("dh_absdiff_up4_combine", P(partial), P(a), P(b), P(da), P(db), N, H, W, S())
    return da, db


def absdiff(a, b):
    y = torch.empty_like(a)
    _call("dh_absdiff", dt(a), P(a), P(b), P(y), a.numel(), S())
    return y


def absdiff_bwd(a, b, dy, da, db, accumulate=True):
    _call("dh_absdiff_bwd", dt(a), P(a), P(b), P(dy), P(da), P(db), a.numel(), accumulate, S())


def colsum(x2d, out, accumulate=False):
    C = x2d.shape[-1]
    Pn = x2d.numel() // C
    ws = workspace(1024 * C * 4 + 1024, x2d.device)
    _call("dh_colsum", dt(x2d), P(x2d), Pn, C, P(out), accumulate, P(ws), S())


def cast_from_f32(src, dtype):
    dst = torch.empty(src.shape, dtype=dtype, device=src.device)
    _call("dh_cast_from_f32", _DT[dtype], P(src), P(dst), src.numel(), S())
    return dst


def cast_to_f32(src, dst=None, accumulate=False):
    if dst is None:
        dst = torch.empty(src.shape, dtype=torch.float32, device=src.device)
    _call("dh_cast_to_f32", dt(src), P(src), P(dst), src.numel(), accumulate, S())
    return dst


def tokenizer_fwd(x, wa, pos, B, L):
    Sn, H, W, C = x.shape
    HW = H * W
    dev = x.device
    logits = torch.empty(Sn * HW, L, dtype=torch.float32, device=dev)
    stats = torch.empty(Sn, L, 2, dtype=torch.float32, device=dev)
    pooled = torch.empty(Sn, L, 32, dtype=torch.float32, device=dev)
    tok = torch.empty(B, 2 * L, 32, dtype=torch.float32, device=dev)
    nws = _lib.lib().dh_tokenizer_fwd_workspace_size(Sn, HW, L)
    args = lambda ws: (dt(x), P(x), P(wa), P(pos), Sn, B, HW, L, P(logits), P(stats), P(pooled), P(tok), P(ws), S())
    if _XPREP_BATCH is not None and _ENC_BATCH is not None:
        ws = torch.empty(max(int(nws), 1), dtype=torch.uint8, device=dev)
        _XPREP_BATCH.extend((ws, x, pos))
        _call("dh_tokenizer_fwd", *args(ws))
    else:
        with _XprepPaused():
# ... 373 lines not shown
    y = torch.empty_like(x2d)
    _call("dh_softmax_groups_fwd", dt(x2d), P(x2d), P(y), rows, heads, L, HLP, S())
    return y


def softmax_groups_bwd(y, dy, heads, L):
    rows, HLP = y.shape
    dx = torch.empty_like(y)
    _call("dh_softmax_groups_bwd", dt(y), P(y), P(dy), P(dx), rows, heads, L, HLP, S())
    return dx


def self_attn(qkv, B, n, heads, dim_head, scale=32 ** -0.5):
    inner = heads * dim_head
    o = torch.empty(B * n, inner, dtype=qkv.dtype, device=qkv.device)
    attn = torch.empty(B, heads, n, n, dtype=torch.float32, device=qkv.device)
    _call("dh_self_attn_fwd", dt(qkv), P(qkv), P(o), P(attn), B, n, heads, dim_head, scale, S())
    return o, attn


def self_attn_bwd(qkv, attn, dout, B, n, heads, dim_head, scale=32 ** -0.5):
    dqkv = torch.empty_like(qkv)
    _call("dh_self_attn_bwd", dt(qkv), P(qkv), P(attn), P(dout), P(dqkv), B, n, heads, dim_head, scale, S())
    return dqkv


def focal_loss(logits_nchw, target, want_grad=True, grad_scale=1.0, alpha=0.5):
    B, C, H, W = logits_nchw.shape
    loss = torch.empty((), dtype=torch.float32, device=logits_nchw.device)
    dl = torch.empty_like(logits_nchw) if want_grad else None
    ws = workspace(4096, logits_nchw.device)
    _call("dh_focal_loss", P(logits_nchw), P(target), B, C, H * W, alpha, grad_scale, P(loss), P(dl), P(ws), S())
    return loss, dl


def cross_entropy_fwd(logits_nchw, target, ignore_index=255):
    B, C, H, W = logits_nchw.shape
    out = torch.empty(2, dtype=torch.float32, device=logits_nchw.device)
    ws = workspace(16384, logits_nchw.device)
    _call("dh_cross_entropy_fwd", P(logits_nchw), P(target), B, C, H * W, ignore_index, P(out), P(ws), S())
    return out


def cross_entropy_bwd(logits_nchw, target, fwd_out, upstream, ignore_index=255):
    B, C, H, W = logits_nchw.shape
    dl = torch.empty_like(logits_nchw)
    _call("dh_cross_entropy_bwd", P(logits_nchw), P(target), B, C, H * W, ignore_index, P(fwd_out), P(upstream), P(dl), S())
    return dl


def dice_argmax_constant(logits_nchw, target, eps=1e-7):
    B, C, H, W = logits_nchw.shape
    loss = torch.empty((), dtype=torch.float32, device=logits_nchw.device)
    ws = workspace(24576, logits_nchw.device)
    _call("dh_dice_argmax_constant", P(logits_nchw), P(target), B, C, H * W, eps, P(loss), P(ws), S())
    return loss


def confusion_matrix(logits_nchw, target, counts, want_mask=False):
    B, C, H, W = logits_nchw.shape
    mask = torch.empty(B, H, W, dtype=torch.int64, device=logits_nchw.device) if want_mask else None
    _call("dh_confusion_matrix", P(logits_nchw), P(target), B, C, H * W, P(mask), P(counts), S())
    return mask


def argmax_nchw(logits_nchw):
# ... 237 lines not shown
```

include/dahitra_hip.h:

```cpp
#ifndef DAHITRA_HIP_H
#define DAHITRA_HIP_H
#ifdef __cplusplus
extern "C" {
#endif

#define DH_F32 0
#define DH_BF16 1
#define DH_ACT_NONE 0
#define DH_ACT_RELU 1
#define DH_ACT_GELU 2

int dh_abi_version(void);
const char* dh_last_error(void);
void dh_set_error(const char* msg);

int dh_conv2d_fwd(int dtype, const void* x, const void* w_packed, void* y, const float* bias,
                  const void* residual, float* stats_partial, int N, int H, int W, int Cin, int OH, int OW,
                  int Cout, int CoutPad, int ks, int stride, int pad, int act, int npix_valid,
                  long w_image_stride, void* y_preact, int dilation, const void* gate_out, const void* gate_y,
                  const float* gate_mean, const float* gate_invstd, int gate_groups, const float* in_scale,
                  const float* in_shift, int in_groups, int phase_mode, const void* w_frag, void* stream);
int dh_conv2d_fwd_num_tiles(int dtype, int N, int OH, int OW, int Cin, int ks, int stride);
int dh_conv2d_fwd_describe(int entry, int dtype, int N, int H, int W, int Cin, int OH, int OW, int Cout, int CoutPad, int ks, int stride,
                           int pad, int act, int npix_valid, long w_image_stride, int dilation, int gate_groups, int in_groups,
// ... 6 lines not shown
int dh_absdiff_up4_combine(const float* partial, const void* a, const void* b, void* da, void* db, int N, int H, int W, void* stream);
int dh_conv3x3_head_fwd(int dtype, const void* x, const void* w_packed, const float* bias, int N, int H, int W, int Cin,
                        int Cout, const float* in_scale, const float* in_shift, int in_groups, float* logits_nchw, void* stream);

int dh_conv2d_wgrad(int dtype, const void* x, const void* dy, float* dw_oihw, int accumulate, int N, int H,
                    int W, int Cin, int OH, int OW, int Cout, int ks, int stride, int pad, int groups,
                    int npix_valid, int use_tr, int Cout_real, int cin_pitch, int dilation, void* workspace, void* stream);
int dh_conv2d_wgrad_1x1_blocks(int N, int H, int W, int Cin, int Cout);
int dh_conv2d_wgrad_describe(int dtype, int accumulate, int N, int H, int W, int Cin, int OH, int OW, int Cout, int ks, int stride,
                             int pad, int groups, int npix_valid, int use_tr, int Cout_real, int cin_pitch, int dilation,
                             int in_groups, int has_in_scale, int split_input, int batch_open, int* out);
long dh_conv2d_wgrad_workspace_size(int N, int OH, int OW, int Cin, int Cout, int ks, int groups);
int dh_conv2d_wgrad_partial(int dtype, const void* x, const void* dy, float* dw_oihw, int accumulate, int N, int H,
                            int W, int Cin, int OH, int OW, int Cout, int ks, int stride, int pad, int groups,
                            int npix_valid, int use_tr, int Cout_real, int cin_pitch, int dilation, void* workspace,
                            int* splitk_out, void* stream);
int dh_conv2d_wgrad_bn_in(int dtype, const void* x, const void* dy, float* dw_oihw, int accumulate, int N, int H, int W,
                          int Cin, int OH, int OW, int Cout, int ks, int stride, int pad, int use_tr, int Cout_real,
                          int dilation, const float* in_scale, const float* in_shift, int in_groups, void* workspace,
                          int* splitk_out, void* stream);
int dh_conv3x3_split_supported(int N, int H, int W, int Cin, int Cout);
int dh_conv3x3_split_fwd(const void* x, long x_split_bytes, const void* w_packed, const void* w_frag, void* y, long y_split_bytes,
                         float* stats_partial, int N, int H, int W, int Cin, int Cout, void* stream);
int dh_conv2d_wgrad_split(const void* x, long x_split_bytes, const void* dy, float* dw_oihw, int accumulate, int N, int H, int W,
                          int Cin, int Cout, void* workspace, int* splitk_out, void* stream);
int dh_conv3x3_up4_fwd(const void* a, const void* b, const void* w_packed, const float* bias, int act, void* y, float* stats_partial,
                       int N, int H, int W, void* stream);
int dh_wgrad_batch_begin(void);
int dh_wgrad_batch_pending(void);
int dh_wgrad_batch_launch(void* stream);
int dh_wgrad_batch_end(void* stream);
int dh_wgrad_batch_abort(void);
int dh_wgrad_reduce_multi(const void* jobs_dev, int njobs, int total_blocks, void* stream);
int dh_pack_phase_weights(int dtype, const float* w_oihw, const float* bias, int Cin, void* fwd, void* dgrad, float* bias4,
                          void* stream);
long dh_conv2d_wgrad_phase_workspace_size(int N, int H, int W, int Cin);
int dh_conv2d_wgrad_phase(int dtype, const void* x, const void* dy, int N, int H, int W, int Cin, int use_tr, void* workspace,
                          int* splitk_out, void* stream);
int dh_phase_wgrad_combine(const float* dwab, float* dw_oihw, int Cin, int accumulate, void* stream);
int dh_pack_s2_dgrad_phase_weights(int dtype, const float* w_oihw, int Co, int Ci, void* out, void* stream);
int dh_wgrad_reduce_job_size(void);
int dh_wgrad_reduce_outputs_per_block(int Cin);
int dh_conv2d_wgrad_splitk(int N, int OH, int OW, int Cin, int Cout, int ks, int groups);

int dh_pack_weight(int dtype, const float* w_oihw, const float* out_scale, int O, int I, int ks, int OPad, void* fwd, int IPad,
                   int dgrad_inner, void* dgrad, void* stream);
int dh_pack_weights_multi(const void* jobs_dev, int njobs, int total_blocks, void* stream);
int dh_pack_job_size(void);
int dh_zero_insert2(int dtype, const void* dy, void* z, int N, int OH, int OW, int H, int W, int C, void* stream);
int dh_add_coarse(int dtype, void* x, const void* coarse, int N, int OH, int OW, int H, int W, int C, void* stream);

int dh_stem_space_to_depth(int dtype, const float* x_nchw, void* y, int N, int H, int W, int CP, void* stream);
int dh_stem_pack_weight(int dtype, const float* w_oihw, const float* out_scale, void* packed, int O, int CP, void* stream);
int dh_stem_unpack_grad(const float* dw2, float* dw_oihw, int O, int CP, int accumulate, void* stream);
int dh_stem7_fwd(const float* xa, const float* xb, int B, int N, int H, int W, const float* w_oihw, const float* out_scale,
                 const float* bias, int relu, void* y, float* stats, int groups, void* xs16, void* stream);
int dh_stem7_fwd_num_slots(int N, int H, int W, int groups);
long dh_stem_pool_bn_bwd_workspace_size(int C, int groups);
int dh_stem_pool_bn_bwd(const unsigned char* argmax, const void* dpool, const void* y, const float* mask_scale,
                        const float* mask_shift, const float* mean, const float* invstd, const float* gamma, int N, int H, int W,
                        int C, int groups, void* d, float* coef, float* dgamma, float* dbeta, int accumulate, void* workspace,
                        void* stream);
int dh_stem_pool_bn_bwd_plus(const unsigned char* argmax, const void* dpool, const void* extra, const void* y,
                             const float* mask_scale, const float* mask_shift, const float* mean, const float* invstd,
                             const float* gamma, int N, int H, int W, int C, int groups, void* d, float* coef, float* dgamma,
                             float* dbeta, int accumulate, void* workspace, void* stream);
int dh_stem_wgrad_bn(const void* xs16, const void* d, const void* y, const float* coef, int groups, int N, int OH, int OW,
                     float* dw2, int use_tr, void* workspace, void* stream);

int dh_bn_finalize(const float* partial, int ntiles, int CP, int C, int groups, double count, const float* gamma,
                   const float* beta, float* running_mean, float* running_var, float momentum, float eps,
                   float* mean, float* invstd, float* scale, float* shift, long long* num_batches_tracked,
                   void* stream);
int dh_bn_eval_params(const float* gamma, const float* beta, const float* running_mean, const float* running_var,
                      float eps, int C, float* scale, float* shift, void* stream);
int dh_bn_apply(int dtype, const void* x, const void* residual, void* y, const float* scale, const float* shift,
                long npix, int C, int groups, int act, void* stream);
int dh_bn_bwd(int dtype, const void* dout, const void* out_relu, const void* x, const float* mean,
              const float* invstd, const float* gamma, long npix, int C, int groups, void* dx, void* dres,
              float* dgamma, float* dbeta, int accumulate, const float* mask_scale, const float* mask_shift,
              void* workspace, void* stream);
// ... 50 lines not shown
                        void* stream);
int dh_head_bn_bwd_blocks(int N, int H, int W, int groups);
long dh_head_bn_bwd_workspace_size(int N, int H, int W, int groups);
int dh_head_dlogits_pack(int dtype, const float* dlogits_nchw, int N, int NC, int H, int W, void* dlp, void* stream);
int dh_head_bn_bwd(int dtype, const void* dlp, const float* w_oihw, int NC, const void* y, const float* mask_scale, const float* mask_shift,
                   const float* mean, const float* invstd, const float* gamma, int groups, void* dx, float* dgamma, float* dbeta,
                   float* dw, float* db, int accumulate, int N, int H, int W, void* workspace, void* stream);
int dh_head_relu_bwd(int dtype, const void* dlp, const float* w_oihw, int NC, const void* relu_out, void* dx, float* dw, float* db,
                     int accumulate, int N, int H, int W, void* workspace, void* stream);
int dh_head_fwd_supported(int NC, int W);
int dh_head_fwd(int dtype, const void* x, const float* w_oihw, const float* bias, int NC, const float* in_scale, const float* in_shift,
                int in_groups, float* logits_nchw, int N, int H, int W, void* stream);
enum { DH_EW_ADD_POS = 1, DH_EW_CAT_HALVES = 2, DH_EW_SPLIT_HALVES = 3, DH_EW_ABSDIFF_HALVES = 4, DH_EW_ABSDIFF_HALVES_BWD = 5,
       DH_EW_ADD_POS_BWD = 6 };
int dh_ew_multi(int n, const int* op, const void* const* a, const void* const* b, void* const* c, const int* i0, const int* i1,
                const long* l0, void* stream);
int dh_nhwc_to_nchw(int dtype, const void* src, float* dst, int N, int C, long HW, void* stream);
int dh_copy_channels(int dtype, const void* src, int Cs, int sc0, void* dst, int Cd, int dc0, int Cn, long P, void* stream);
int dh_cat_halves(int dtype, void* t, void* cat, int C, long P, int inverse, void* stream);
int dh_add(int dtype, const void* a, const void* b, void* y, long n, void* stream);
int dh_add_pos(int dtype, const void* x, const float* pos, void* y, int N, long HW, int C, void* stream);
int dh_add_pos_bwd(int dtype, const void* dy, float* dpos, int N, long HW, int C, int accumulate, void* stream);
int dh_act_bwd(int dtype, const void* dy, const void* ref, void* dx, long n, int act, void* stream);
int dh_maxpool3x3s2_fwd(int dtype, const void* x, void* y, unsigned char* argmax, int N, int H, int W, int C,
                        const float* bn_scale, const float* bn_shift, int groups, void* stream);
int dh_maxpool3x3s2_bwd(int dtype, const unsigned char* argmax, const void* dy, void* dx, int N, int H, int W, int C, void* stream);
int dh_upsample2_nearest_fwd(int dtype, const void* x, void* y, int N, int H, int W, int C, void* stream);
int dh_upsample2_nearest_bwd(int dtype, const void* dy, void* dx, int N, int H, int W, int C, void* stream);
int dh_absdiff_upsample4_fwd(int dtype, const void* a, const void* b, void* y, int N, int H, int W, int C, void* stream);
int dh_absdiff_upsample4_bwd(int dtype, const void* a, const void* b, const void* dy, void* da, void* db, int N, int H, int W, int C, void* stream);
int dh_absdiff(int dtype, const void* a, const void* b, void* y, long n, void* stream);
int dh_absdiff_bwd(int dtype, const void* a, const void* b, const void* dy, void* da, void* db, long n, int accumulate, void* stream);
int dh_colsum(int dtype, const void* x, long P, int C, float* out, int accumulate, void* workspace, void* stream);
int dh_cast_from_f32(int dtype, const float* src, void* dst, long n, void* stream);
int dh_cast_to_f32(int dtype, const void* src, float* dst, long n, int accumulate, void* stream);

int dh_tokenizer_fwd(int dtype, const void* x, const float* wa, const float* pos, int S, int B, int HW, int L,
                     float* logits, float* stats, float* pooled, float* tok_cat, void* workspace, void* stream);
long dh_tokenizer_fwd_workspace_size(int S, int HW, int L);
int dh_tokenizer_bwd(int dtype, const void* x, const float* wa, int S, int B, int HW, int L, const float* logits,
                     const float* stats, const float* pooled, const float* dtok_cat, void* dx_accum, float* dwa,
                     float* dpos, int accumulate, void* workspace, void* stream);
long dh_tokenizer_bwd_workspace_size(int S, int HW, int L);
int dh_xattn_prep_fwd(int dtype, const void* tok, long tok_bstride, long tok_sstride, int B, int S, int L, int heads,
                      int dim_head, int HLP, float scale, float eps, const float* ln_g, const float* ln_b,
                      const float* wq, const void* wkT, const void* wvT, const void* woT, float* mn, float* mstats,
                      float* k, float* v, void* kq, void* kqT, void* vo, void* voT, void* stream);
int dh_xattn_prep_fwd_stack(int dtype, const void* tok, long tok_bstride, long tok_sstride, int B, int S, int L, int heads,
                            int dim_head, int HLP, float scale, float eps, int layers, long param_stride,
                            const float* ln_g, const float* ln_b, const float* wq, const void* wkT, const void* wvT,
                            const void* woT, float* mn, float* mstats, float* k, float* v, void* kq, void* kqT, void* vo,
                            void* voT, void* stream);
int dh_xattn_prep_mfma_supported(int dtype, int S, int L, int heads, int dim_head, int HLP);
int dh_xattn_prep_fwd_stack_mfma(const void* tok, long tok_bstride, long tok_sstride, int B, int S, int heads, int dim_head,
                                 int HLP, float scale, float eps, int layers, long param_stride, const float* ln_g,
                                 const float* ln_b, const float* wk, const float* wv, const float* wo, const void* wqT,
                                 float* mn, float* mstats, float* k, float* v, void* kq, void* kqT, void* vo, void* voT,
                                 void* stream);
int dh_xattn_prep_bwd_stack_mfma(const void* tok, void* dtok_accum, long tok_bstride, long tok_sstride, int B, int S, int heads,
                                 int dim_head, int HLP, float scale, int layers, long param_stride, const float* ln_g,
                                 const float* wq, const void* woT, const void* wkT, const void* wvT, const float* mn,
                                 const float* mstats, const float* k, const float* v, const float* dkq, const float* dvoT,
                                 float* dk, float* dv, float* dln_g, float* dln_b, float* dwq, float* dwk, float* dwv,
                                 float* dwo, int accumulate, void* workspace, void* stream);
int dh_xattn_prep_bwd_stack(int dtype, const void* tok, void* dtok_accum, long tok_bstride, long tok_sstride, int B, int S,
                            int L, int heads, int dim_head, int HLP, float scale, int layers, long param_stride,
// ... 48 lines not shown
int dh_decoder_layer_fwd(const void* x, void* y, const void* kq, const void* voT, const float* ln1_g,
                         const float* ln1_b, const float* bo, const float* ln2_g, const float* ln2_b, const void* w1,
                         const float* b1, const void* w2, const float* b2, long rows, int rows_per_image, int mlp,
                         float eps, void* stream);
int dh_decoder_layer_fwd_fp8(const void* x, void* y, const void* kq, const void* voT, const float* ln1_g,
                         const float* ln1_b, const float* bo, const float* ln2_g, const float* ln2_b, const void* w1,
                         const float* b1, const void* w2, const float* b2, long rows, int rows_per_image, int mlp,
                         float eps, void* stream);
int dh_decoder_layer_bwd(const void* x, const void* dy, void* dx, const void* kq, const void* voT, const void* vo,
                         const void* kqT, const float* ln1_g, const float* ln1_b, const float* bo, const float* ln2_g,
                         const float* ln2_b, const void* w1, const void* w1T, const float* b1, const void* w2,
                         const void* w2T, const float* b2, float* dw1, float* dw2, float* db1, float* db2, float* dbo,
                         float* dln1_g, float* dln1_b, float* dln2_g, float* dln2_b, float* dkq, float* dvoT, long rows,
                         int rows_per_image, int mlp, float eps, void* workspace, void* stream);
int dh_decoder_stack_fwd(const void* x, void* ys, const void* kq, const void* voT, const float* ln1_g, const float* ln1_b,
                         const float* bo, const float* ln2_g, const float* ln2_b, const void* w1, const float* b1, const void* w2,
                         const float* b2, int depth, long kq_lstride, long w_lstride, long par_lstride, long rows,
                         int rows_per_image, int mlp, float eps, void* stream);
int dh_decoder_stack_bwd(const void* x, const void* ys, const void* dy, void* dx, void* dwork, const void* kq, const void* voT,
                         const void* vo, const void* kqT, const float* ln1_g, const float* ln1_b, const float* bo,
                         const float* ln2_g, const float* ln2_b, const void* w1, const void* w1T, const float* b1, const void* w2,
                         const void* w2T, const float* b2, int depth, long kq_lstride, long w_lstride, long par_lstride, long rows,
                         int rows_per_image, int mlp, float eps, void* workspace, void* stream);
int dh_decoder_stack_bwd_finalize(const void* workspace, int depth, long rows, int rows_per_image, int mlp, float* dw1, float* dw2,
                                  float* db1, float* db2, float* dbo, float* dln1_g, float* dln1_b, float* dln2_g, float* dln2_b,
                                  long grad_stride, float* dkq, float* dvoT, void* stream);
long dh_decoder_layer_bwd_workspace_size(long rows, int rows_per_image, int mlp);
int dh_decoder_plan_describe(int backward, int stack, int mlp, int batch_open, int njobs, const long* rows, const int* rows_per_image,
                             const int* depth, int cus, long* out);

int dh_focal_loss(const float* logits_nchw, const long long* target, int B, int C, long HW, float alpha,
                  float grad_scale, float* loss_out, float* dlogits_nchw, void* workspace, void* stream);
int dh_argmax_nchw(const float* logits_nchw, long long* mask, int B, int C, long HW, void* stream);
int dh_cross_entropy_fwd(const float* logits_nchw, const long long* target, int B, int C, long HW, int ignore_index,
                         float* out_dev, void* workspace, void* stream);
int dh_cross_entropy_bwd(const float* logits_nchw, const long long* target, int B, int C, long HW, int ignore_index,
                         const float* fwd_out_dev, const float* upstream_dev, float* dlogits_nchw, void* stream);
int dh_dice_argmax_constant(const float* logits_nchw, const long long* target, int B, int C, long HW, float eps,
                            float* loss_out, void* workspace, void* stream);
int dh_adamw_step_graph(float* param, const float* grad, float* exp_avg, float* exp_avg_sq, long n,
                        float* hyper_dev, int* step_dev, void* stream);
int dh_confusion_matrix(const float* logits_nchw, const long long* target, int B, int C, long HW, long long* mask,
                        long long* counts, void* stream);
int dh_scale_by_scalar(const float* src, const float* scalar_dev, float* dst, long n, void* stream);
int dh_absdiff_halves(int dtype, const void* tok, void* out, int B, long n, void* stream);
int dh_absdiff_halves_bwd(int dtype, const void* tok, const void* dout, void* dtok_accum, int B, long n, void* stream);
int dh_adamw_step(float* param, const float* grad, float* exp_avg, float* exp_avg_sq, long n, float lr, float beta1,
                  float beta2, float eps, float weight_decay, int step, float grad_scale, void* stream);


long dh_combo_loss_workspace_size(int C);
int dh_combo_loss_fwd(const float* logits, const float* masks, int B, int C, long HW, const float* weights_dev,
                      float dice_weight, float focal_weight, float* sums_out, float* channel_loss_out, float* loss_out,
                      void* workspace, void* stream);
int dh_combo_loss_bwd(const float* logits, const float* masks, const float* sums, const float* weights_dev,
                      const float* upstream_dev, float dice_weight, float focal_weight, int B, int C, long HW,
                      float* dlogits, void* stream);
long dh_grad_norm_workspace_size(void);
int dh_grad_norm_clip_coef(const float* grad, long n, float max_norm, float* out_dev, void* workspace, void* stream);
int dh_adamw_xbd_step(float* param, const float* grad, float* exp_avg, float* exp_avg_sq, long n, float lr, float beta1,
                      float beta2, float eps, float weight_decay, int step, const float* grad_scale_dev, void* stream);
int dh_adamw_xbd_step_graph(float* param, const float* grad, float* exp_avg, float* exp_avg_sq, long n, float* hyper_dev,
                            int* step_dev, const float* grad_scale_dev, void* stream);

int dh_xbd_val_count(const float* logits, const unsigned char* msk0, long msk0_image_stride, const unsigned char* lbl, int B,
                     int H, int W, float thr, int select, long long* image_counts, long long* class_counts, void* stream);
// ... 15 lines not shown
```

Before: 9747 image-pairs/s.

## Fold stem, phase-combine and colsum reductions into one multi-kind wgrad reduce launch

Adds a second multi-job wgrad reduce kernel whose jobs carry a kind tag (slab, stem, phase-combine, column-sum), so the stem weight-gradient unpack, the four-phase combine and bias column sums finish inside one batched launch instead of separate kernels. Focal loss gains a packed path that writes the 2-class gradient as padded bf16 pairs, with an optional ticket-based last-block reduction of the loss. Weight packing and combine code move into shared device helpers. The aim is fewer small kernel launches and intermediate buffers in the graphed step, at the cost of a more complex job table and a busier reduction kernel.

```diff
diff --git a/dahitra_amd/csrc/conv_wgrad.hip b/dahitra_amd/csrc/conv_wgrad.hip
--- a/dahitra_amd/csrc/conv_wgrad.hip
+++ b/dahitra_amd/csrc/conv_wgrad.hip
@@ -1,4 +1,5 @@
 #include "common.h"
+#include "phase_pack.h"
 
 namespace {
 
@@ -588,6 +589,106 @@
     const WgReduceJob job = jobs[j];
     wgrad_reduce_block(job.part, job.splitk, job.taps, job.Oslab, job.O, job.I, job.dw, job.accumulate,
                        (long)blockIdx.x - job.first_block, red);
+}
+
+__device__ __forceinline__ float wgrad_reduce_phase(const float* __restrict__ src, int splitk, size_t slab, int ph) {
+    float a0 = 0.f, a1 = 0.f, a2 = 0.f, a3 = 0.f;
+    int k = ph;
+    for (; k + 24 < splitk; k += 32) {
+        a0 += src[(size_t)k * slab];
+        a1 += src[(size_t)(k + 8) * slab];
+        a2 += src[(size_t)(k + 16) * slab];
+        a3 += src[(size_t)(k + 24) * slab];
+    }
+    for (; k < splitk; k += 8) a0 += src[(size_t)k * slab];
+    return (a0 + a1) + (a2 + a3);
+}
+__device__ __forceinline__ void phase_wgrad_combine_store(const float (&v)[4][4], float* __restrict__ dw, int i, int accumulate) {
+    const int ra[3][2] = {{0, 1}, {0, 1}, {0, 1}}, rt[3][2] = {{0, 0}, {1, 0}, {1, 1}};
+#pragma unroll
+    for (int kh = 0; kh < 3; ++kh)
+#pragma unroll
+        for (int kw = 0; kw < 3; ++kw) {
+            float s = 0.f;
+#pragma unroll
+            for (int m = 0; m < 2; ++m)
+#pragma unroll
+                for (int n = 0; n < 2; ++n) s += v[ra[kh][m] * 2 + ra[kw][n]][rt[kh][m] * 2 + rt[kw][n]];
+            float* d = dw + (size_t)i * 9 + kh * 3 + kw;
+            if (accumulate) *d += s; else *d = s;
+        }
+}
+struct WgReduceJob2 {
+    const float* part;
+    float* dw;
+    int splitk, taps, Oslab, O, I, accumulate, first_block, nblocks;
+    int kind, reserved;
+};
+enum { WGR_SLAB = 0, WGR_STEM = 1, WGR_COMBINE = 2, WGR_COLSUM = 3 };
+__device__ __forceinline__ void wgrad_stem_block(const WgReduceJob2& j, int block, float (*red)[32]) {
+    const int lane = threadIdx.x & 31, ph = threadIdx.x >> 5;
+    const int i = block * 32 + lane, n = j.O * 147;
+    float v = 0.f;
+    if (i < n) {
+        const int kw = i % 7, kh = (i / 7) % 7, c = (i / 49) % 3, o = i / 147;
+        const int dy = (kh + 1) / 2, ry = (kh + 1) % 2, dx = (kw + 1) / 2, rx = (kw + 1) % 2;
+        const int ch = (ry * 2 + rx) * 3 + c, tap = dy * 4 + dx;
+        v = wgrad_reduce_phase(j.part + ((size_t)tap * j.Oslab + o) * j.I + ch, j.splitk, (size_t)16 * j.Oslab * j.I, ph);
+    }
+    red[ph][lane] = v;
+    __syncthreads();
+    if (ph == 0 && i < n) {
+        float s = 0.f;
+#pragma unroll
+        for (int r = 0; r < 8; ++r) s += red[r][lane];
+        if (j.accumulate) j.dw[i] += s; else j.dw[i] = s;
+    }
+}
+__device__ __forceinline__ void wgrad_combine_block(const WgReduceJob2& j, int block, float* lds ) {
+    const int lane = threadIdx.x & 31, ph = threadIdx.x >> 5;
+    const int i = block * 32 + lane, n = 32 * j.I;
+    const size_t slab = (size_t)4 * 32 * j.I, per = (size_t)j.splitk * slab;
+#pragma unroll 4
+    for (int q = 0; q < 16; ++q)
+        lds[(ph * 16 + q) * 32 + lane] = i < n ? wgrad_reduce_phase(j.part + (size_t)(q >> 2) * per + (size_t)(q & 3) * 32 * j.I + i, j.splitk, slab, ph) : 0.f;
+    __syncthreads();
+    float f[2];
+#pragma unroll
+    for (int e = 0; e < 2; ++e) {
+        float s = 0.f;
+#pragma unroll
+        for (int r = 0; r < 8; ++r) s += lds[(r * 16 + 2 * ph + e) * 32 + lane];
+        f[e] = s;
+    }
+    __syncthreads();
+    lds[(2 * ph) * 32 + lane] = f[0];
+    lds[(2 * ph + 1) * 32 + lane] = f[1];
+    __syncthreads();
+    if (ph == 0 && i < n) {
+        float v[4][4];
+#pragma unroll
+        for (int q = 0; q < 16; ++q) v[q >> 2][q & 3] = lds[q * 32 + lane];
+        phase_wgrad_combine_store(v, j.dw, i, j.accumulate);
+    }
+}
+__global__ __launch_bounds__(256) __attribute__((amdgpu_waves_per_eu(8, 8))) void wgrad_reduce_multi2_kernel(const WgReduceJob2* __restrict__ jobs, int njobs) {
+    __shared__ __attribute__((aligned(16))) float lds[8 * 16 * 32];
+    int lo = 0, hi = njobs - 1;
+    while (lo < hi) {
+        const int mid = (lo + hi + 1) >> 1;
+        if (jobs[mid].first_block <= (int)blockIdx.x) lo = mid; else hi = mid - 1;
+    }
+    const WgReduceJob2 job = jobs[lo];
+    const int local = (int)blockIdx.x - job.first_block;
+    if (local >= job.nblocks) return;
+    if (job.kind == WGR_SLAB)
+        wgrad_reduce_block(job.part, job.splitk, job.taps, job.Oslab, job.O, job.I, job.dw, job.accumulate, local,
+                           reinterpret_cast<float(*)[132]>(lds));
+    else if (job.kind == WGR_STEM) wgrad_stem_block(job, local, reinterpret_cast<float(*)[32]>(lds));
+    else if (job.kind == WGR_COMBINE) wgrad_combine_block(job, local, lds);
+    else if (job.kind == WGR_COLSUM)
+        dh_reduce_partials_body(job.part, (long)job.splitk, (long)job.I, 1.0f, job.dw, job.accumulate, local,
+                                reinterpret_cast<double(*)[32]>(lds));
 }
 
 #ifdef DH_WS_TIMING
@@ -1322,6 +1423,22 @@
     DH_CHECK_LAUNCH("wgrad_reduce_multi");
     return 0;
 }
+extern "C" int dh_wgrad_reduce_job2_size(void) { return (int)sizeof(WgReduceJob2); }
+extern "C" int dh_wgrad_reduce_multi2(const void* jobs_dev, int njobs, int total_blocks, void* stream) {
+    if (njobs <= 0) return 0;
+    DH_REQUIRE(jobs_dev && total_blocks > 0, "wgrad_reduce_multi2: empty table");
+    hipLaunchKernelGGL(wgrad_reduce_multi2_kernel, dim3(total_blocks), dim3(256), 0, reinterpret_cast<hipStream_t>(stream),
+                       reinterpret_cast<const WgReduceJob2*>(jobs_dev), njobs);
+    DH_CHECK_LAUNCH("wgrad_reduce_multi2");
+    return 0;
+}
+extern "C" int dh_stem_wgrad_bn_partial(const void* xs16, const void* d, const void* y, const float* coef, int groups, int N, int OH,
+                                        int OW, float* dw2, int use_tr, void* workspace, int* splitk_out, void* stream) {
+    DH_REQUIRE(xs16 && d && y && coef && splitk_out && workspace && groups >= 1 && N % groups == 0,
+               "stem_wgrad_bn_partial: bad arguments (N=%d groups=%d)", N, groups);
+    return conv2d_wgrad_impl(DH_DTYPE_BF16, xs16, d, dw2, 0, N, OH, OW, 16, OH, OW, 64, 4, 1, 2, 1, 0, use_tr, 0, 16, 1, workspace,
+                             stream, 1, splitk_out, nullptr, nullptr, 1, y, coef, groups);
+}
 
 extern "C" long dh_conv2d_wgrad_phase_workspace_size(int N, int H, int W, int Cin) {
     WgArgs a = wg_args(N, H, W, Cin, H, W, 32, 1);
@@ -1350,72 +1467,20 @@
         const float4 q = *reinterpret_cast<const float4*>(src + ph * pstride);
         v[ph][0] = q.x; v[ph][1] = q.y; v[ph][2] = q.z; v[ph][3] = q.w;
     }
-    const int ra[3][2] = {{0, 1}, {0, 1}, {0, 1}}, rt[3][2] = {{0, 0}, {1, 0}, {1, 1}};
-#pragma unroll
-    for (int kh = 0; kh < 3; ++kh)
-#pragma unroll
-        for (int kw = 0; kw < 3; ++kw) {
-            float s = 0.f;
-#pragma unroll
-            for (int m = 0; m < 2; ++m)
-#pragma unroll
-                for (int n = 0; n < 2; ++n) s += v[ra[kh][m] * 2 + ra[kw][n]][rt[kh][m] * 2 + rt[kw][n]];
-            float* d = dw + (size_t)i * 9 + kh * 3 + kw;
-            if (accumulate) *d += s; else *d = s;
-        }
+    phase_wgrad_combine_store(v, dw, i, accumulate);
 }
 
 template <typename T>
 __global__ void pack_phase_weights_kernel(const float* __restrict__ w, const float* __restrict__ bias, int Cin,
                                           T* __restrict__ fwd, T* __restrict__ dgrad, float* __restrict__ bias4) {
-    const int i = blockIdx.x * blockDim.x + threadIdx.x;
-    if (i < 128 && bias4) bias4[i] = bias ? bias[i & 31] : 0.f;
-    if (i >= 32 * Cin) return;
-    const int co = i / Cin, ci = i % Cin;
-    float k[3][3];
-#pragma unroll
-    for (int j = 0; j < 9; ++j) k[j / 3][j % 3] = w[(size_t)i * 9 + j];
-    const int lo[2][2] = {{0, 1}, {0, 2}}, hi[2][2] = {{0, 2}, {1, 2}};
-#pragma unroll
-    for (int a = 0; a < 2; ++a)
-#pragma unroll
-        for (int b = 0; b < 2; ++b)
-#pragma unroll
-            for (int t = 0; t < 2; ++t)
-#pragma unroll
-                for (int u = 0; u < 2; ++u) {
-                    float s = 0.f;
-                    for (int kh = lo[a][t]; kh <= hi[a][t]; ++kh)
-                        for (int kw = lo[b][u]; kw <= hi[b][u]; ++kw) s += k[kh][kw];
-                    const int ph = a * 2 + b;
-                    if (fwd) stf(fwd + ((size_t)(t * 2 + u) * 128 + ph * 32 + co) * Cin + ci, s);
-                    if (dgrad) stf(dgrad + ((size_t)((1 - t) * 2 + (1 - u)) * Cin + ci) * 128 + ph * 32 + co, s);
-                }
+    pack_phase_weights_body<T>(w, bias, Cin, fwd, dgrad, bias4, blockIdx.x * blockDim.x + threadIdx.x);
 }
 }
 
 namespace {
 template <typename T>
 __global__ void pack_s2_dgrad_phase_kernel(const float* __restrict__ w, int Co, int Ci, T* __restrict__ out) {
-    const int i = blockIdx.x * blockDim.x + threadIdx.x;
-    if (i >= Co * Ci) return;
-    const int co = i / Ci, ci = i % Ci;
-    float k[3][3];
-#pragma unroll
-    for (int j = 0; j < 9; ++j) k[j / 3][j % 3] = w[(size_t)i * 9 + j];
-    const int kmap[2][2] = {{-1, 1}, {2, 0}};
-#pragma unroll
-    for (int a = 0; a < 2; ++a)
-#pragma unroll
-        for (int b = 0; b < 2; ++b)
-#pragma unroll
-            for (int t = 0; t < 2; ++t)
-#pragma unroll
-                for (int u = 0; u < 2; ++u) {
-                    const int kh = kmap[a][t], kw = kmap[b][u];
-                    const float v = (kh >= 0 && kw >= 0) ? k[kh][kw] : 0.f;
-                    stf(out + ((size_t)(t * 2 + u) * 4 * Ci + (a * 2 + b) * Ci + ci) * Co + co, v);
-                }
+    pack_s2_dgrad_phase_body<T>(w, Co, Ci, out, blockIdx.x * blockDim.x + threadIdx.x);
 }
 }
 extern "C" int dh_pack_s2_dgrad_phase_weights(int dtype, const float* w_oihw, int Co, int Ci, void* out, void* stream) {
diff --git a/dahitra_amd/csrc/loss_optim.hip b/dahitra_amd/csrc/loss_optim.hip
--- a/dahitra_amd/csrc/loss_optim.hip
+++ b/dahitra_amd/csrc/loss_optim.hip
@@ -7,8 +7,10 @@
 template <int CT>
 __global__ __launch_bounds__(256) void focal_kernel(const float* __restrict__ logits, const long long* __restrict__ target,
                                                     int B, int Crt, long HW, float alpha, float gscale,
-                                                    float* __restrict__ dlogits, float* __restrict__ partial) {
-    __shared__ float red[256];
+                                                    float* __restrict__ dlogits, float* partial, unsigned* dlp,
+                                                    int W, unsigned* ticket, float lscale, float* __restrict__ loss_out) {
+    __shared__ double red64[8][32];
+    float* red = reinterpret_cast<float*>(red64);
     const int C = CT > 0 ? CT : Crt;
     constexpr int NC = CT > 0 ? CT : MAXC;
     const long total = (long)B * HW;
@@ -17,6 +19,7 @@
     const long i0 = (long)blockIdx.x * blockDim.x + threadIdx.x;
     long b = i0 / HW, p = i0 - b * HW;
     const long db = stride / HW, dp = stride - db * HW;
+    const long Hp = (CT == 2 && dlp) ? HW / W + 2 : 0;
     for (long i = i0; i < total; i += stride) {
         float z[NC], pr[NC], lp[NC];
         float m = -INFINITY;
@@ -43,9 +46,25 @@
             }
         lsum += loss;
         if (dlogits) {
+            float g[NC];
 #pragma unroll
             for (int c = 0; c < NC; ++c)
-                if (c < C) dlogits[(b * C + c) * HW + p] = gscale * (gp[c] - pr[c] * gsum);
+                if (c < C) g[c] = gscale * (gp[c] - pr[c] * gsum);
+            bool packed = false;
+            if constexpr (CT == 2) {
+                if (dlp) {
+                    packed = true;
+                    const unsigned y = (unsigned)p / (unsigned)W, x = (unsigned)p - y * (unsigned)W;
+                    float g0 = g[0], g1 = g[1];
+                    asm volatile("" : "+v"(g0), "+v"(g1));
+                    dlp[(b * Hp + y + 1) * (W + 2) + x + 1] = f2bf2(g0, g1);
+                }
+            }
+            if (!packed) {
+#pragma unroll
+                for (int c = 0; c < NC; ++c)
+                    if (c < C) dlogits[(b * C + c) * HW + p] = g[c];
+            }
         }
         b += db; p += dp;
         if (p >= HW) { p -= HW; ++b; }
@@ -56,7 +75,26 @@
         if (threadIdx.x < o) red[threadIdx.x] += red[threadIdx.x + o];
         __syncthreads();
     }
-    if (threadIdx.x == 0) partial[blockIdx.x] = red[0];
+    if constexpr (CT == 2) {
+        if (!ticket) {
+            if (threadIdx.x == 0) partial[blockIdx.x] = red[0];
+            return;
+        }
+        __shared__ unsigned last;
+        if (threadIdx.x == 0) {
+            __hip_atomic_store(&partial[blockIdx.x], red[0], __ATOMIC_RELAXED, __HIP_MEMORY_SCOPE_AGENT);
+            asm volatile("s_waitcnt vmcnt(0)" ::: "memory");
+            last = __hip_atomic_fetch_add(ticket, 1u, __ATOMIC_RELAXED, __HIP_MEMORY_SCOPE_AGENT) == gridDim.x - 1;
+        }
+        __syncthreads();
+        if (last) {
+            __builtin_amdgcn_fence(__ATOMIC_ACQUIRE, "agent");
+            dh_reduce_partials_body(partial, (long)gridDim.x, 1L, lscale, loss_out, 0, 0, red64);
+            if (threadIdx.x == 0) __hip_atomic_store(ticket, 0u, __ATOMIC_RELAXED, __HIP_MEMORY_SCOPE_AGENT);
+        }
+    } else {
+        if (threadIdx.x == 0) partial[blockIdx.x] = red[0];
+    }
 }
 
 __global__ __launch_bounds__(256) void ce_partial_kernel(const float* __restrict__ logits, const long long* __restrict__ target,
@@ -246,9 +284,25 @@
     float* partial = reinterpret_cast<float*>(workspace);
     auto kern = C == 2 ? focal_kernel<2> : (C == 5 ? focal_kernel<5> : focal_kernel<0>);
     hipLaunchKernelGGL(kern, dim3((int)g), dim3(256), 0, ST(stream), logits_nchw, target, B, C, HW, alpha,
-                       grad_scale / (float)total, dlogits_nchw, partial);
+                       grad_scale / (float)total, dlogits_nchw, partial, (unsigned*)nullptr, 0, (unsigned*)nullptr, 0.f,
+                       (float*)nullptr);
     DH_CHECK_LAUNCH("focal_loss");
     return dh_reduce_partials(partial, g, 1, 1.0f / (float)total, loss_out, 0, stream);
+}
+
+extern "C" int dh_focal_loss_packed(const float* logits_nchw, const long long* target, int B, int C, int H, int W, float alpha,
+                                    float grad_scale, float* loss_out, void* dlp, void* workspace, void* ticket, void* stream) {
+    DH_REQUIRE(C == 2, "focal_loss_packed: n_class=%d unsupported (2: the bf16 pair map of the change-detection heads)", C);
+    DH_REQUIRE(B > 0 && H > 0 && W > 0 && logits_nchw && target && loss_out && dlp && workspace, "focal_loss_packed: empty input");
+    DH_REQUIRE((long)B * (H + 2) * (W + 2) * 8 < (1L << 31), "focal_loss_packed: %d x %d x %d does not fit a 2 GiB buffer descriptor", B, H, W);
+    const long total = (long)B * H * W;
+    long g = (total + 255) / 256;
+    if (g > 1024) g = 1024;
+    hipLaunchKernelGGL(focal_kernel<2>, dim3((int)g), dim3(256), 0, ST(stream), logits_nchw, target, B, C, (long)H * W, alpha,
+                       grad_scale / (float)total, reinterpret_cast<float*>(dlp), reinterpret_cast<float*>(workspace),
+                       reinterpret_cast<unsigned*>(dlp), W, reinterpret_cast<unsigned*>(ticket), 1.0f / (float)total, loss_out);
+    DH_CHECK_LAUNCH("focal_loss_packed");
+    return ticket ? 0 : dh_reduce_partials(reinterpret_cast<float*>(workspace), g, 1, 1.0f / (float)total, loss_out, 0, stream);
 }
 
 extern "C" int dh_cross_entropy_fwd(const float* logits_nchw, const long long* target, int B, int C, long HW,
diff --git a/dahitra_amd/csrc/phase_pack.h b/dahitra_amd/csrc/phase_pack.h
--- /dev/null
+++ b/dahitra_amd/csrc/phase_pack.h
@@ -0,0 +1,51 @@
+#pragma once
+#include "common.h"
+
+template <typename T>
+__device__ __forceinline__ void pack_phase_weights_body(const float* __restrict__ w, const float* __restrict__ bias, int Cin,
+                                                        T* __restrict__ fwd, T* __restrict__ dgrad, float* __restrict__ bias4, int i) {
+    if (i < 128 && bias4) bias4[i] = bias ? bias[i & 31] : 0.f;
+    if (i >= 32 * Cin) return;
+    const int co = i / Cin, ci = i % Cin;
+    float k[3][3];
+#pragma unroll
+    for (int j = 0; j < 9; ++j) k[j / 3][j % 3] = w[(size_t)i * 9 + j];
+    const int lo[2][2] = {{0, 1}, {0, 2}}, hi[2][2] = {{0, 2}, {1, 2}};
+#pragma unroll
+    for (int a = 0; a < 2; ++a)
+#pragma unroll
+        for (int b = 0; b < 2; ++b)
+#pragma unroll
+            for (int t = 0; t < 2; ++t)
+#pragma unroll
+                for (int u = 0; u < 2; ++u) {
+                    float s = 0.f;
+                    for (int kh = lo[a][t]; kh <= hi[a][t]; ++kh)
+                        for (int kw = lo[b][u]; kw <= hi[b][u]; ++kw) s += k[kh][kw];
+                    const int ph = a * 2 + b;
+                    if (fwd) stf(fwd + ((size_t)(t * 2 + u) * 128 + ph * 32 + co) * Cin + ci, s);
+                    if (dgrad) stf(dgrad + ((size_t)((1 - t) * 2 + (1 - u)) * Cin + ci) * 128 + ph * 32 + co, s);
+                }
+}
+
+template <typename T>
+__device__ __forceinline__ void pack_s2_dgrad_phase_body(const float* __restrict__ w, int Co, int Ci, T* __restrict__ out, int i) {
+    if (i >= Co * Ci) return;
+    const int co = i / Ci, ci = i % Ci;
+    float k[3][3];
+#pragma unroll
+    for (int j = 0; j < 9; ++j) k[j / 3][j % 3] = w[(size_t)i * 9 + j];
+    const int kmap[2][2] = {{-1, 1}, {2, 0}};
+#pragma unroll
+    for (int a = 0; a < 2; ++a)
+#pragma unroll
+        for (int b = 0; b < 2; ++b)
+#pragma unroll
+            for (int t = 0; t < 2; ++t)
+#pragma unroll
+                for (int u = 0; u < 2; ++u) {
+                    const int kh = kmap[a][t], kw = kmap[b][u];
+                    const float v = (kh >= 0 && kw >= 0) ? k[kh][kw] : 0.f;
+                    stf(out + ((size_t)(t * 2 + u) * 4 * Ci + (a * 2 + b) * Ci + ci) * Co + co, v);
+                }
+}
diff --git a/dahitra_amd/csrc/pointwise.hip b/dahitra_amd/csrc/pointwise.hip
--- a/dahitra_amd/csrc/pointwise.hip
+++ b/dahitra_amd/csrc/pointwise.hip
@@ -1,4 +1,5 @@
 #include "common.h"
+#include "phase_pack.h"
 
 namespace {
 
@@ -971,6 +972,55 @@
     if ((j.dtype & 0xff) == DH_DTYPE_BF16) pack_job<bf16>(j, lb); else pack_job<float>(j, lb);
 }
 
+struct PrologueJob {
+    const float* w;
+    void* fwd;
+    void* dgrad;
+    void* aux;
+    const float* bias;
+    long bytes;
+    int O, I, KS, OPad, IPad, OK;
+    int dtype, first_block, nblocks, kind;
+};
+enum { PRO_PACK = 0, PRO_PHASE = 1, PRO_S2_PHASE = 2, PRO_ZERO = 3 };
+__device__ __forceinline__ void zero_job(const PrologueJob& j, int lb) {
+    const long n16 = j.bytes >> 4;
+    uint4* d = reinterpret_cast<uint4*>(j.fwd);
+    for (long q = (long)lb * blockDim.x + threadIdx.x; q < n16; q += (long)j.nblocks * blockDim.x) d[q] = make_uint4(0u, 0u, 0u, 0u);
+    const int tail = (int)(j.bytes & 15);
+    if (lb == 0 && (int)threadIdx.x < tail) reinterpret_cast<unsigned char*>(j.fwd)[(n16 << 4) + threadIdx.x] = 0;
+}
+__global__ __launch_bounds__(256) void step_prologue_multi_kernel(const PrologueJob* __restrict__ jobs, int njobs) {
+    int lo = 0, hi = njobs - 1;
+    while (lo < hi) {
+        const int mid = (lo + hi + 1) >> 1;
+        if (jobs[mid].first_block <= (int)blockIdx.x) lo = mid; else hi = mid - 1;
+    }
+    const PrologueJob j = jobs[lo];
+    const int lb = blockIdx.x - j.first_block;
+    if (lb >= j.nblocks) return;
+    __shared__ __attribute__((aligned(16))) float tile[PK_T * PK_PITCH];
+    const bool b16 = (j.dtype & 0xff) == DH_DTYPE_BF16;
+    if (j.kind == PRO_PACK) {
+        const PackJob pj = {j.w, j.fwd, j.dgrad, j.O, j.I, j.KS, j.OPad, j.IPad, j.OK, j.dtype, j.first_block, j.nblocks};
+        if (pack_tiled(pj)) {
+            if (b16) pack_job_tiled<bf16>(pj, lb, tile); else pack_job_tiled<float>(pj, lb, tile);
+        } else {
+            if (b16) pack_job<bf16>(pj, lb); else pack_job<float>(pj, lb);
+        }
+    } else if (j.kind == PRO_PHASE) {
+        const int i = lb * 256 + (int)threadIdx.x;
+        if (b16) pack_phase_weights_body<bf16>(j.w, j.bias, j.I, (bf16*)j.fwd, (bf16*)j.dgrad, (float*)j.aux, i);
+        else pack_phase_weights_body<float>(j.w, j.bias, j.I, (float*)j.fwd, (float*)j.dgrad, (float*)j.aux, i);
+    } else if (j.kind == PRO_S2_PHASE) {
+        const int i = lb * 256 + (int)threadIdx.x;
+        if (b16) pack_s2_dgrad_phase_body<bf16>(j.w, j.O, j.I, (bf16*)j.fwd, i);
+        else pack_s2_dgrad_phase_body<float>(j.w, j.O, j.I, (float*)j.fwd, i);
+    } else if (j.kind == PRO_ZERO) {
+        zero_job(j, lb);
+    }
+}
+
 template <typename T>
 __global__ __launch_bounds__(256) void colsum_partial_kernel(const T* __restrict__ x, long P, int C,
                                                              float* __restrict__ partial) {
@@ -1300,6 +1350,15 @@
     return 0;
 }
 extern "C" int dh_pack_job_size(void) { return (int)sizeof(PackJob); }
+extern "C" int dh_step_prologue_job_size(void) { return (int)sizeof(PrologueJob); }
+extern "C" int dh_step_prologue_multi(const void* jobs_dev, int njobs, int total_blocks, void* stream) {
+    if (njobs <= 0) return 0;
+    DH_REQUIRE(jobs_dev && total_blocks > 0, "step_prologue_multi: empty table");
+    hipLaunchKernelGGL(step_prologue_multi_kernel, dim3(total_blocks), dim3(256), 0, ST(stream),
+                       reinterpret_cast<const PrologueJob*>(jobs_dev), njobs);
+    DH_CHECK_LAUNCH("step_prologue_multi");
+    return 0;
+}
 extern "C" int dh_pack_weights_multi(const void* jobs_dev, int njobs, int total_blocks, void* stream) {
     if (njobs <= 0) return 0;
     hipLaunchKernelGGL(pack_weights_multi_kernel, dim3(total_blocks), dim3(256), 0, ST(stream),
@@ -1307,16 +1366,21 @@
     DH_CHECK_LAUNCH("pack_weights_multi");
     return 0;
 }
-extern "C" int dh_colsum(int dtype, const void* x, long P, int C, float* out, int accumulate, void* workspace, void* stream) {
-    DH_REQUIRE(C >= 1 && C <= 256, "colsum: C=%d out of range", C);
+extern "C" int dh_colsum_partial(int dtype, const void* x, long P, int C, float* partial, int* rows_out, void* stream) {
+    DH_REQUIRE(C >= 1 && C <= 256 && partial && rows_out, "colsum: C=%d out of range", C);
     const long rows_per_pass = 256 / (C >= 4 && (C & 3) == 0 ? C / 4 : C);
     long want = (P + rows_per_pass * 8 - 1) / (rows_per_pass * 8);
     const int grid = (int)(want < 64 ? 64 : (want > 256 ? 256 : want));
-    float* partial = reinterpret_cast<float*>(workspace);
     if (dtype == DH_DTYPE_BF16) hipLaunchKernelGGL(colsum_partial_kernel<bf16>, dim3(grid), dim3(256), 0, ST(stream), (const bf16*)x, P, C, partial);
     else hipLaunchKernelGGL(colsum_partial_kernel<float>, dim3(grid), dim3(256), 0, ST(stream), (const float*)x, P, C, partial);
     DH_CHECK_LAUNCH("colsum");
-    return dh_reduce_partials(partial, grid, C, 1.0f, out, accumulate, stream);
+    *rows_out = grid;
+    return 0;
+}
+extern "C" int dh_colsum(int dtype, const void* x, long P, int C, float* out, int accumulate, void* workspace, void* stream) {
+    int grid = 0;
+    if (const int rc = dh_colsum_partial(dtype, x, P, C, reinterpret_cast<float*>(workspace), &grid, stream)) return rc;
+    return dh_reduce_partials(reinterpret_cast<float*>(workspace), grid, C, 1.0f, out, accumulate, stream);
 }
 extern "C" int dh_cast_from_f32(int dtype, const float* src, void* dst, long n, void* stream) {
     if (dtype == DH_DTYPE_BF16) hipLaunchKernelGGL(cast_from_f32_kernel<bf16>, dim3(ew_grid(n, 256)), dim3(256), 0, ST(stream), src, (bf16*)dst, n);
diff --git a/dahitra_amd/engine.py b/dahitra_amd/engine.py
--- a/dahitra_amd/engine.py
+++ b/dahitra_amd/engine.py
@@ -94,6 +94,18 @@
         self._bwd = None
         self._plans = {}
         self._wgrad_plan = None
+        self.step_grad = None
+        self.step_zeroed = False
+        self._zbufs = {}
+        self.loss_packed = False
+        self._dlp = {}
+
+    def focal_loss_packed(self, logits, target):
+        N, _, H, W = logits.shape
+        buf = self._dlp.get((N, H, W))
+        if buf is None:
+            buf = self._dlp[(N, H, W)] = ops.head_dlp_buffer(N, H, W, logits.device)
+        return ops.focal_loss_packed(logits, target, buf[0], buf[1] if ops.GLUE_TICKET else None)
 
     def bind(self, params, grads):
         self.p, self.g = params, grads
@@ -104,16 +116,37 @@
         if plan is None:
             plan = self._plans[self.need_grad] = self._build_plan()
         pack, self.pk, self.xstack, self.wstack = plan
+        step = ops.STEP_GLUE and self.need_grad and self.step_grad is not None
+        if step and not pack.zeroes(self.step_grad, step_only=True):
+            pack.add_zero(self.step_grad, step_only=True)
+        self.step_zeroed = step
         if self.pack_side and self.training and self.direct_stem and self.dtype == torch.bfloat16 and ops.PROFILE is None:
             if self._pack_stream is None:
                 self._pack_stream = ops.SideStream(self.p["resnet.conv1.weight"].device)
             with self._pack_stream.fork():
-                pack.run()
+                pack.run(step=step)
         else:
-            pack.run()
+            pack.run(step=step)
         key = "resnet.conv1.weight"
         if not (self.direct_stem and self.dtype == torch.bfloat16):
             self.pk[key] = Packed(ops.stem_pack_weight(self.p[key], self.dtype), None)
+
+    def take_step_zeroed(self):
+        z, self.step_zeroed = self.step_zeroed, False
+        return z
+
+    def _step_zeros(self, name, shape, dtype, device):
+        if not (ops.STEP_GLUE and self.step_grad is not None):
+            return torch.zeros(shape, dtype=dtype, device=device)
+        key = (name, tuple(shape), dtype, str(device))
+        buf = self._zbufs.get(key)
+        if buf is None:
+            buf = self._zbufs[key] = torch.empty(shape, dtype=dtype, device=device)
+        pack = self._plans[True][0]
+        if not pack.zeroes(buf):
+            pack.add_zero(buf)
+            buf.zero_()
+        return buf
 
     def _pack_join(self):
         if self._pack_stream is not None:
@@ -133,9 +166,13 @@
                     key.startswith("resnet.layer4"):
                 continue
             if key == "conv_pred.weight" and self.phase_conv_pred and shape[1] % 64 == 0 and self.cfg["kind"] == "bit":
+                if ops.STEP_GLUE:
+                    pk[key + ":phase"] = pack.add_phase(self.p[key], self.p["conv_pred.bias"], self.dtype)
                 continue
             if self.phase_up_conv and key in ("conv_layer2.0.weight", "conv_layer3.0.weight", "conv_layer4.0.weight") and \
                     tuple(shape[:2]) == (32, 32):
+                if ops.STEP_GLUE:
+                    pk[key + ":phase"] = pack.add_phase(self.p[key], self.p[key[:-len("weight")] + "bias"], self.dtype)
                 continue
             if ".to_q." in key or ".to_k." in key or ".to_v." in key or \
                     (".to_out." in key and "transformer_decoder" in key):
@@ -189,7 +226,13 @@
             assert ks == 1 and stride == 2 and residual is None and gate is None
             return ops.conv2d(dy, self.pk[wkey].dgrad, Cin, 1, 1, 0, alg_flops=flops)
         if gate is None and self.s2_phase_ok(ks, stride, pad, xshape, dy):
-            wph = ops.pack_s2_dgrad_phase_weights(self.p[wkey], self.dtype)
+            wph = self.pk.get(wkey + ":s2phase")
+            if wph is None:
+                if ops.STEP_GLUE and self._plans.get(True) is not None and self.pk is self._plans[True][1]:
+                    wph = self.pk[wkey + ":s2phase"] = self._plans[True][0].add_s2_phase(self.p[wkey], self.dtype)
+                    ops.pack_s2_dgrad_phase_weights(self.p[wkey], self.dtype, out=wph)
+                else:
+                    wph = ops.pack_s2_dgrad_phase_weights(self.p[wkey], self.dtype)
             if residual is None or isinstance(residual, CoarseRes):
                 return ops.conv3x3s2_dgrad(dy, wph, Cin, residual.t if residual is not None else None, alg_flops=flops)
             return ops.add(ops.conv3x3s2_dgrad(dy, wph, Cin, None, alg_flops=flops), residual)
@@ -281,21 +324,21 @@
             dy = ops.act_bwd(dout, out, RELU) if (act == RELU and not masked) else dout
             ops.conv2d_wgrad(x, dy, self.g[wkey], ks, 1, pad, accumulate=True, use_tr=self.use_tr)
             if bkey:
-                ops.colsum(dy.view(-1, cout), self.g[bkey], accumulate=True)
+                ops.colsum(dy.view(-1, cout), self.g[bkey], accumulate=True, defer=True)
             dx = self.conv_dgrad(dy, wkey, ks, 1, pad, x.shape, residual=dx_res) if need_dx else None
             return dx
         return out, bwd
 
     def conv_pred_phase(self, x):
         wkey, bkey = "conv_pred.weight", "conv_pred.bias"
-        wf, wd, b4 = ops.pack_phase_weights(self.p[wkey], self.p[bkey], self.dtype)
+        wf, wd, b4 = self.pk.get(wkey + ":phase") or ops.pack_phase_weights(self.p[wkey], self.p[bkey], self.dtype)
         out = ops.conv_up2_fwd(x, wf, b4)
         if not self.need_grad:
             return out, None
 
         def bwd(dout):
             ops.conv_up2_wgrad(x, dout, self.g[wkey], accumulate=True, use_tr=self.use_tr)
-            ops.colsum(dout.view(-1, 32), self.g[bkey], accumulate=True)
+            ops.colsum(dout.view(-1, 32), self.g[bkey], accumulate=True, defer=True)
             return ops.conv_up2_dgrad(dout, wd, x.shape[-1])
         return out, bwd
 
@@ -760,6 +803,8 @@
     def forward(self, x1, x2, training, need_grad):
         ops.set_f32_mma_mode(self.mma_fwd)
         self.training, self.need_grad = training, need_grad
+        if need_grad:
+            self.loss_packed = False
         if need_grad and self.use_side and self.side is None and self.dtype == torch.bfloat16:
             self.side = ops.SideStream(x1.device)
         self._pack_all()
@@ -857,14 +902,26 @@
         small = 8 if (self.dtype == torch.bfloat16 or ncls > 4) else 4
         direct = h.shape[-1] == 32 and ncls <= small
 
+        def fuses():
+            return self.fused_head_bn and ncls <= 8 and self.g[wkey].is_contiguous() and \
+                (self.dtype == torch.bfloat16 or (self.dtype == torch.float32 and ops.get_f32_mma_mode() != 0))
+
+        def takes_packed(next_gate=None, head_bn=None, relu_out=None):
+            return ops.STEP_GLUE and direct and next_gate is None and ncls <= 2 and self.dtype == torch.bfloat16 and fuses() and \
+                (head_bn is not None or (relu_out is not None and relu_out is h))
+
+        def pack(dl_nchw):
+            return dl_nchw.dlp if isinstance(dl_nchw, ops.PackedDlogits) else ops.head_dlogits_pack(dl_nchw, self.dtype)
+
         def bwd(dl_nchw, next_gate=None, head_bn=None, relu_out=None):
+            if isinstance(dl_nchw, ops.PackedDlogits) and not takes_packed(next_gate, head_bn, relu_out):
+                raise RuntimeError("dahitra_amd: a packed loss gradient reached a class head that needs the fp32 one")
             if direct and next_gate is None:
-                fuse = self.fused_head_bn and ncls <= 8 and self.g[wkey].is_contiguous() and \
-                    (self.dtype == torch.bfloat16 or (self.dtype == torch.float32 and ops.get_f32_mma_mode() != 0))
+                fuse = fuses()
                 if head_bn is not None and fuse:
-                    return HeadGrad(ops.head_dlogits_pack(dl_nchw, self.dtype), self.p[wkey], ncls, self.g[wkey], self.g[bkey])
+                    return HeadGrad(pack(dl_nchw), self.p[wkey], ncls, self.g[wkey], self.g[bkey])
                 if relu_out is not None and fuse and relu_out is h:
-                    return ops.head_relu_bwd(ops.head_dlogits_pack(dl_nchw, self.dtype), self.p[wkey], ncls, h, self.g[wkey],
+                    return ops.head_relu_bwd(pack(dl_nchw), self.p[wkey], ncls, h, self.g[wkey],
                                              self.g[bkey])
                 dl = ops.nchw_to_nhwc(dl_nchw, self.dtype, cpad=small)
                 ops.conv2d_wgrad(h, dl, self.g[wkey], 3, 1, 1, accumulate=True, use_tr=self.use_tr, cout_real=ncls)
@@ -881,6 +938,7 @@
             ops.reduce_rows(tmp, 1, ncls, self.g[bkey], accumulate=True)
             dh = self.conv_dgrad(dl, wkey, 3, 1, 1, h.shape, gate=next_gate)
             return ops.act_bwd(dh, relu_out, RELU) if relu_out is not None else dh
+        bwd.takes_packed = takes_packed
         return out, bwd
 
     def _bit(self, x1, x2):
@@ -909,7 +967,7 @@
         tok_cat, tsaved = ops.tokenizer_fwd(feat, wa, self.p["pos_embedding"], B, L)
         tok2d, b_enc = self.encoder(tok_cat.view(B * 2 * L, DIM), "transformer", cfg["enc_depth"], BIT_HEADS,
                                     BIT_DIM_HEAD, B, 2 * L)
-        dtok = torch.zeros_like(tok2d) if self.need_grad else None
+        dtok = self._step_zeros("dtok", tok2d.shape, tok2d.dtype, tok2d.device) if self.need_grad else None
         dec, b_dec = self.decoder(feat.view(S2 * hw, DIM), S2, tok2d, 2 * L * DIM, L * DIM, B, dtok,
                                   "transformer_decoder", cfg["dec_depth"], BIT_HEADS, cfg["dec_dim_head"], L)
         dec4 = dec.view(S2, fh, fw, DIM)
@@ -923,6 +981,7 @@
         logits, b_out = self._head_out(h, "classifier.3.weight", "classifier.3.bias")
         if not self.need_grad:
             return logits, None
+        self.loss_packed = b_out.takes_packed(next_gate=b_c0.gate, head_bn=getattr(b_c0, "bn", None))
 
         def bwd_first(dl):
             dh = b_out(dl, next_gate=b_c0.gate, head_bn=getattr(b_c0, "bn", None))
@@ -1094,7 +1153,7 @@
             if not self.need_grad:
                 return out, None
             return out, (lambda d, masked=False: ops.upsample2_bwd(b(d, masked=masked)))
-        wf, wd, b4 = ops.pack_phase_weights(self.p[wkey], self.p[bkey], self.dtype)
+        wf, wd, b4 = self.pk.get(wkey + ":phase") or ops.pack_phase_weights(self.p[wkey], self.p[bkey], self.dtype)
         out = ops.conv_up2_fwd(x, wf, b4, act=RELU)
         if not self.need_grad:
             return out, None
@@ -1102,7 +1161,7 @@
         def bwd(dout, masked=False):
             dy = dout if masked else ops.act_bwd(dout, out, RELU)
             ops.conv_up2_wgrad(x, dy, self.g[wkey], accumulate=True, use_tr=self.use_tr)
-            ops.colsum(dy.view(-1, 32), self.g[bkey], accumulate=True)
+            ops.colsum(dy.view(-1, 32), self.g[bkey], accumulate=True, defer=True)
             return ops.conv_up2_dgrad(dy, wd, 32)
         return out, bwd
 
@@ -1117,7 +1176,7 @@
         s16, b_l3 = self.res_layer(p16, 3, 1, 2)
         level = self._xbd_level if self.cfg["kind"] == "xbd" else self._level
         if self.need_grad:
-            self._zpool = [torch.zeros(3 * 3 * B * self.cfg["token_len"] * DIM, dtype=torch.float32, device=s4.device), 0]
+            self._zpool = [self._step_zeros("zpool", (3 * 3 * B * self.cfg["token_len"] * DIM,), torch.float32, s4.device), 0]
         ew = self.cfg["kind"] != "xbd"
         (o5, b5), (t4, b4), (t3, b3) = self._run_staged([level(5, s16, B), level(4, s8, B), level(3, s4, B)], ew=ew)
         self._zpool = None
@@ -1137,12 +1196,13 @@
         logits, b_out = self._head_out(o2, "classifier.weight", "classifier.bias")
         if not self.need_grad:
             return logits, None
+        self.loss_packed = b_out.takes_packed(relu_out=o2)
 
         def bwd_first(dl):
             do2 = b_out(dl, relu_out=o2)
             dy2 = bu2(do2, masked=True)
             ops.conv2d_wgrad(y, dy2, self.g["conv_layer2_0.3.weight"], 3, 1, 1, accumulate=True, use_tr=self.use_tr)
-            ops.colsum(dy2.view(-1, 32), self.g["conv_layer2_0.3.bias"], accumulate=True)
+            ops.colsum(dy2.view(-1, 32), self.g["conv_layer2_0.3.bias"], accumulate=True, defer=True)
             dy = self.conv_dgrad(dy2, "conv_layer2_0.3.weight", 3, 1, 1, y.shape, gate=b20.gate)
             dcat2, _ = b20(dy)
             if split2:
diff --git a/dahitra_amd/graph.py b/dahitra_amd/graph.py
--- a/dahitra_amd/graph.py
+++ b/dahitra_amd/graph.py
@@ -92,24 +92,36 @@
         if type(self)._eager_body is not GraphedTrainStep._eager_body or os.environ.get("DAHITRA_GRAPH_AUTOGRAD") == "1":
             return self._eager_body(include_opt)
         net = self.net
-        logits = self._forward_split()
+        logits = self._forward_zeroing()
         bwd = net._engine.take_backward()
         self.logits = logits
         loss, dl = self._loss_and_grad(logits)
         self._count(logits)
-        net._arena.grad.zero_()
+        if not net._engine.take_step_zeroed():
+            net._arena.grad.zero_()
         net._engine.backward(dl, bwd)
         net._bind_grad_views()
         if include_opt:
             self.opt.step()
         return loss
 
+    def _forward_zeroing(self):
+        eng = self.net._engine
+        eng.step_grad = self.net._arena.grad if ops.STEP_GLUE else None
+        try:
+            return self._forward_split()
+        finally:
+            eng.step_grad = None
+
     def _forward_split(self):
         return self.net._run_forward(self.a, self.b, need_grad=True)
 
     def _loss_and_grad(self, logits):
         tgt = self.lab[:, 0] if self.lab.dim() == logits.dim() else self.lab
-        return ops.focal_loss(logits, tgt.to(torch.int64).contiguous(), want_grad=True)
+        tgt = tgt.to(torch.int64).contiguous()
+        if self.net._engine.loss_packed:
+            return self.net._engine.focal_loss_packed(logits, tgt)
+        return ops.focal_loss(logits, tgt, want_grad=True)
 
     def _count(self, logits):
         if self.confusion is not None:
@@ -122,12 +134,13 @@
 
     def _split_first(self):
         net = self.net
-        logits = self._forward_split()
+        logits = self._forward_zeroing()
         bwd = net._engine.take_backward()
         self.logits = logits
         loss, dl = self._loss_and_grad(logits)
         self._count(logits)
-        net._arena.grad.zero_()
+        if not net._engine.take_step_zeroed():
+            net._arena.grad.zero_()
         net._engine.backward_first(dl, bwd)
         net._bind_grad_views()
         return loss
diff --git a/dahitra_amd/ops.py b/dahitra_amd/ops.py
--- a/dahitra_amd/ops.py
+++ b/dahitra_amd/ops.py
@@ -87,10 +87,11 @@
     if eng._wgrad_plan is not None:
         keep += list(eng._wgrad_plan.slots) + list(eng._wgrad_plan.tables.values())
     for pack, _, xstack, wstack in eng._plans.values():
-        keep += [pack.table] + list(pack.keep) + list(xstack.values())
+        keep += [pack.table, pack.ptable] + list(pack.keep) + list(xstack.values())
         for fwd_stack, dgrad_stack in wstack.values():
             keep += [fwd_stack, dgrad_stack]
     keep += [net._arena.flat, net._arena.grad]
+    keep += [t for pair in eng._dlp.values() for t in pair]
     keep = [t for t in keep if t is not None]
     _PINNED.extend(keep)
     return keep
@@ -134,8 +135,19 @@
                     ("I", ctypes.c_int), ("KS", ctypes.c_int), ("OPad", ctypes.c_int), ("IPad", ctypes.c_int),
                     ("OK", ctypes.c_int), ("dtype", ctypes.c_int), ("first_block", ctypes.c_int), ("nblocks", ctypes.c_int)]
 
+    class _PJob(ctypes.Structure):
+        _fields_ = [("w", ctypes.c_void_p), ("fwd", ctypes.c_void_p), ("dgrad", ctypes.c_void_p), ("aux", ctypes.c_void_p),
+                    ("bias", ctypes.c_void_p), ("bytes", ctypes.c_long), ("O", ctypes.c_int), ("I", ctypes.c_int),
+                    ("KS", ctypes.c_int), ("OPad", ctypes.c_int), ("IPad", ctypes.c_int), ("OK", ctypes.c_int),
+                    ("dtype", ctypes.c_int), ("first_block", ctypes.c_int), ("nblocks", ctypes.c_int), ("kind", ctypes.c_int)]
+
+    PACK, PHASE, S2_PHASE, ZERO = 0, 1, 2, 3
+
     def __init__(self, device):
         self.device, self.jobs, self.blocks, self.table, self.keep = device, [], 0, None, []
+        self.extra = []
+        self.step_zero = []
+        self.ptable, self.counts = None, None
 
     def add(self, w, dtype, want_fwd=True, want_dgrad=True, dgrad_inner=0, out_dgrad=None, frag=False, out_fwd=None):
         if w.dim() == 2:
@@ -163,16 +175,82 @@
                                    _DT[dtype] | (0x200 if frag else 0), self.blocks, nb))
         self.blocks += nb
         self.keep += [w, fwd, dg]
+        self.table = self.ptable = None
         return fwd, dg
 
-    def run(self):
-        if not self.jobs:
+    def add_phase(self, w, bias, dtype, out=None):
+        O, I = w.shape[0], w.shape[1]
+        assert O == 32 and tuple(w.shape[2:]) == (3, 3) and I % 16 == 0 and w.is_contiguous() and (bias is None or bias.is_contiguous())
+        fwd, dg, b4 = out if out is not None else (torch.empty(4, 128, I, dtype=dtype, device=w.device),
+                                                   torch.empty(4, I, 128, dtype=dtype, device=w.device),
+                                                   torch.empty(128, dtype=torch.float32, device=w.device))
+        assert fwd.numel() == dg.numel() == 512 * I and fwd.dtype == dg.dtype == dtype and b4.numel() == 128 and b4.dtype == torch.float32
+        assert fwd.is_contiguous() and dg.is_contiguous() and b4.is_contiguous()
+        self.extra.append(self._PJob(w.data_ptr(), fwd.data_ptr(), dg.data_ptr(), b4.data_ptr(), bias.data_ptr() if bias is not None else None,
+                                     0, 32, I, 3, 0, 0, 0, _DT[dtype], 0, cdiv(32 * I, 256), self.PHASE))
+        self.keep += [w, bias, fwd, dg, b4]
+        self.ptable = None
+        return fwd, dg, b4
+
+    def add_s2_phase(self, w, dtype, out=None):
+        Co, Ci = w.shape[0], w.shape[1]
+        assert Ci in (32, 64) and Co % 16 == 0 and tuple(w.shape[2:]) == (3, 3) and w.is_contiguous()
+        if out is None:
+            out = torch.empty(4, 4 * Ci, Co, dtype=dtype, device=w.device)
+        assert out.numel() == 16 * Ci * Co and out.dtype == dtype and out.is_contiguous()
+        self.extra.append(self._PJob(w.data_ptr(), out.data_ptr(), None, None, None, 0, Co, Ci, 3, 0, 0, 0, _DT[dtype], 0,
+                                     cdiv(Co * Ci, 256), self.S2_PHASE))
+        self.keep += [w, out]
+        self.ptable = None
+        return out
+
+    def add_zero(self, t, step_only=False):
+        nbytes = t.numel() * t.element_size()
+        assert t.is_contiguous() and t.data_ptr() % 16 == 0 and nbytes > 0
+        job = self._PJob(None, t.data_ptr(), None, None, None, nbytes, 0, 0, 0, 0, 0, 0, 0, 0, max(1, min(256, cdiv(nbytes, 1 << 16))),
+                         self.ZERO)
+        (self.step_zero if step_only else self.extra).append(job)
+        self.keep.append(t)
+        self.ptable = None
+
+    def zeroes(self, t, step_only=False):
+        return any(j.kind == self.ZERO and j.fwd == t.data_ptr() and j.bytes == t.numel() * t.element_size()
+                   for j in (self.step_zero if step_only else self.extra))
+
+    def _changed(self):
+        if torch.cuda.is_current_stream_capturing():
+            raise RuntimeError("dahitra_amd: the step prologue's job table changed during graph capture; run one eager step of "
+                               "the same shapes first")
+
+    def run(self, step=False):
+        if not STEP_GLUE:
+            assert not self.extra and not self.step_zero
+            if not self.jobs:
+                return
+            if self.table is None:
+                self._changed()
+                assert ctypes.sizeof(self._Job) == _lib.lib().dh_pack_job_size()
+                raw = b"".join(bytes(j) for j in self.jobs)
+                self.table = torch.frombuffer(bytearray(raw), dtype=torch.uint8).to(self.device)
+            _call("dh_pack_weights_multi", P(self.table), len(self.jobs), self.blocks, S())
             return
-        if self.table is None:
-            assert ctypes.sizeof(self._Job) == _lib.lib().dh_pack_job_size()
-            raw = b"".join(bytes(j) for j in self.jobs)
-            self.table = torch.frombuffer(bytearray(raw), dtype=torch.uint8).to(self.device)
-        _call("dh_pack_weights_multi", P(self.table), len(self.jobs), self.blocks, S())
+        if self.ptable is None:
+            self._changed()
+            assert ctypes.sizeof(self._PJob) == _lib.lib().dh_step_prologue_job_size()
+            recs = [self._PJob(j.w, j.fwd, j.dgrad, None, None, 0, j.O, j.I, j.KS, j.OPad, j.IPad, j.OK, j.dtype, 0, j.nblocks, self.PACK)
+                    for j in self.jobs] + self.extra + self.step_zero
+            blocks, marks = 0, []
+            for k, j in enumerate(recs):
+                if k == len(recs) - len(self.step_zero):
+                    marks = (k, blocks)
+                j.first_block = blocks
+                blocks += j.nblocks
+            self.counts = (marks if self.step_zero else (len(recs), blocks), (len(recs), blocks))
+            if recs:
+                self.ptable = torch.frombuffer(bytearray(b"".join(bytes(j) for j in recs)), dtype=torch.uint8).to(self.device)
+        njobs, blocks = self.counts[1 if step else 0]
+        if njobs:
+            _call("dh_step_prologue_multi", P(self.ptable), njobs, blocks, S())
 
 
 class WgradPlan:
@@ -181,6 +259,13 @@
         _fields_ = [("part", ctypes.c_void_p), ("dw", ctypes.c_void_p), ("splitk", ctypes.c_int), ("taps", ctypes.c_int),
                     ("Oslab", ctypes.c_int), ("O", ctypes.c_int), ("I", ctypes.c_int), ("accumulate", ctypes.c_int),
                     ("first_block", ctypes.c_int), ("nblocks", ctypes.c_int)]
+
+    class _Job2(ctypes.Structure):
+        _fields_ = [("part", ctypes.c_void_p), ("dw", ctypes.c_void_p), ("splitk", ctypes.c_int), ("taps", ctypes.c_int),
+                    ("Oslab", ctypes.c_int), ("O", ctypes.c_int), ("I", ctypes.c_int), ("accumulate", ctypes.c_int),
+                    ("first_block", ctypes.c_int), ("nblocks", ctypes.c_int), ("kind", ctypes.c_int), ("reserved", ctypes.c_int)]
+
+    SLAB, STEM, COMBINE, COLSUM = 0, 1, 2, 3
 
     def __init__(self, device, batch=False):
         self.device, self.slots, self.cur, self.blocks = device, [], 0, 0
@@ -233,11 +318,30 @@
         self.cur += 1
         return buf
 
+    def _add(self, kind, part, dw, splitk, taps, oslab, o, i, accumulate, nb):
+        if GLUE_REDUCE:
+            job = self._Job2(part.data_ptr(), dw.data_ptr(), splitk, taps, oslab, o, i, int(accumulate), self.blocks, nb, kind, 0)
+        else:
+            assert kind == self.SLAB
+            job = self._Job(part.data_ptr(), dw.data_ptr(), splitk, taps, oslab, o, i, int(accumulate), self.blocks, nb)
+        self.jobs.append(job)
+        self.blocks += nb
+
     def add(self, part, dw, splitk, taps, oslab, o, i, accumulate):
-        nb = cdiv(o * i * taps, _lib.lib().dh_wgrad_reduce_outputs_per_block(i))
-        self.jobs.append(self._Job(part.data_ptr(), dw.data_ptr(), splitk, taps, oslab, o, i, int(accumulate),
-                                   self.blocks, nb))
-        self.blocks += nb
+        self._add(self.SLAB, part, dw, splitk, taps, oslab, o, i, accumulate,
+                  cdiv(o * i * taps, _lib.lib().dh_wgrad_reduce_outputs_per_block(i)))
+
+    def add_stem(self, part, dw, splitk, o, accumulate):
+        assert dw.is_contiguous() and dw.numel() == o * 147
+        self._add(self.STEM, part, dw, splitk, 16, o, o, 16, accumulate, cdiv(o * 147, 32))
+
+    def add_combine(self, part, dw, splitk, cin, accumulate):
+        assert dw.is_contiguous() and dw.numel() == 32 * cin * 9
+        self._add(self.COMBINE, part, dw, splitk, 4, 32, 32, cin, accumulate, cin)
+
+    def add_colsum(self, partial, rows, c, out, accumulate):
+        assert out.is_contiguous() and out.numel() == c
+        self._add(self.COLSUM, partial, out, rows, 1, 0, 0, c, accumulate, cdiv(c, 32))
 
     def run(self):
         if self.batching:
@@ -251,17 +355,25 @@
         self.phase += 1
 
     def _run_reduce(self):
+        if GLUE_REDUCE:
+            self.jobs.sort(key=lambda j: j.kind == self.SLAB)
+            blocks = 0
+            for j in self.jobs:
+                j.first_block = blocks
+                blocks += j.nblocks
         sig = b"".join(bytes(j) for j in self.jobs)
         if self.tables.get(self.phase) is None or sig != self.sigs.get(self.phase):
             if torch.cuda.is_current_stream_capturing():
                 raise RuntimeError("dahitra_amd: the weight-gradient plan changed during graph capture; run one eager "
                                    "step of the same shapes first")
             assert ctypes.sizeof(self._Job) == _lib.lib().dh_wgrad_reduce_job_size()
+            assert ctypes.sizeof(self._Job2) == _lib.lib().dh_wgrad_reduce_job2_size()
             if self.tables.get(self.phase) is not None:
                 _PINNED.append(self.tables[self.phase])
             self.tables[self.phase] = torch.frombuffer(bytearray(sig), dtype=torch.uint8).to(self.device)
             self.sigs[self.phase] = sig
-        _call("dh_wgrad_reduce_multi", P(self.tables[self.phase]), len(self.jobs), self.blocks, S())
+        _call("dh_wgrad_reduce_multi2" if GLUE_REDUCE else "dh_wgrad_reduce_multi", P(self.tables[self.phase]), len(self.jobs),
+              self.blocks, S())
 
 
 _WGRAD_PLAN = None
@@ -613,9 +725,11 @@
     return y
 
 
-def pack_s2_dgrad_phase_weights(w, dtype):
+def pack_s2_dgrad_phase_weights(w, dtype, out=None):
     Co, Ci = w.shape[0], w.shape[1]
-    out = torch.empty(4, 4 * Ci, Co, dtype=dtype, device=w.device)
+    if out is None:
+        out = torch.empty(4, 4 * Ci, Co, dtype=dtype, device=w.device)
+    assert tuple(out.shape) == (4, 4 * Ci, Co) and out.dtype == dtype and out.is_contiguous()
     _call("dh_pack_s2_dgrad_phase_weights", _DT[dtype], P(w), Co, Ci, P(out), S())
     return out
 
@@ -651,15 +765,18 @@
         plan.__enter__()
     try:
         ws = plan.slab(L.dh_conv2d_wgrad_phase_workspace_size(N, H, W, Cin))
-        dwab = plan.slab(4 * 32 * Cin * 4 * 4).view(torch.float32)
+        dwab = None if GLUE_STEM_COMBINE else plan.slab(4 * 32 * Cin * 4 * 4).view(torch.float32)
         sk = (ctypes.c_int * 1)()
         with _Prof("conv_wgrad<%s,ks3,s1>" % ("bf16" if x.dtype == torch.bfloat16 else "f32"),
                    2.0 * N * 4 * H * W * 32 * Cin * 9, _nb(x, dy)):
             _call("dh_conv2d_wgrad_phase", dt(x), P(x), P(dy), N, H, W, Cin, use_tr, P(ws), sk, S())
-        per = sk[0] * 4 * 32 * Cin * 4
-        for ph in range(4):
-            plan.add(ws[ph * per:], dwab[ph * 32 * Cin * 4:], sk[0], 4, 32, 32, Cin, False)
-        plan.post.append(lambda: _call("dh_phase_wgrad_combine", P(dwab), P(dw), Cin, accumulate, S()))
+        if GLUE_STEM_COMBINE:
+            plan.add_combine(ws, dw, sk[0], Cin, accumulate)
+        else:
+            per = sk[0] * 4 * 32 * Cin * 4
+            for ph in range(4):
+                plan.add(ws[ph * per:], dwab[ph * 32 * Cin * 4:], sk[0], 4, 32, 32, Cin, False)
+            plan.post.append(lambda: _call("dh_phase_wgrad_combine", P(dwab), P(dw), Cin, accumulate, S()))
         if own:
             plan.run()
     finally:
@@ -747,9 +864,20 @@
         y, coef, groups = bn
         assert cp == 16 and O == 64 and y.shape == dy.shape
         L = _lib.lib()
-        ws = workspace(L.dh_conv2d_wgrad_workspace_size(N, H2, W2, 16, O, 4, 1), dy.device)
-        with _Prof("conv_wgrad<bf16,ks4,s1>", 2.0 * N * H2 * W2 * O * 16 * 16, _nb(x_s2d, dy, y)):
-            _call("dh_stem_wgrad_bn", P(x_s2d), P(dy), P(y), P(coef), groups, N, H2, W2, P(dw2), use_tr, P(ws), S())
+        nbytes = L.dh_conv2d_wgrad_workspace_size(N, H2, W2, 16, O, 4, 1)
+        plan = _WGRAD_PLAN if (GLUE_STEM_COMBINE and PROFILE is None and dw.is_contiguous()) else None
+        if plan is not None:
+            ws = plan.slab(nbytes)
+            sk = (ctypes.c_int * 1)()
+            _call("dh_stem_wgrad_bn_partial", P(x_s2d), P(dy), P(y), P(coef), groups, N, H2, W2, P(dw2), use_tr, P(ws), sk, S())
+            plan.hold(x_s2d, dy, y, coef)
+            if sk[0] > 0:
+                plan.add_stem(ws, dw, sk[0], O, accumulate)
+                return
+        else:
+            ws = workspace(nbytes, dy.device)
+            with _Prof("conv_wgrad<bf16,ks4,s1>", 2.0 * N * H2 * W2 * O * 16 * 16, _nb(x_s2d, dy, y)):
+                _call("dh_stem_wgrad_bn", P(x_s2d), P(dy), P(y), P(coef), groups, N, H2, W2, P(dw2), use_tr, P(ws), S())
     else:
         conv2d_wgrad(x_s2d, dy, dw2, ks=4, stride=1, pad=2, use_tr=use_tr, cin=16, defer=False)
     _call("dh_stem_unpack_grad", P(dw2), P(dw), O, 16, accumulate, S())
@@ -1131,9 +1259,16 @@
     _call("dh_absdiff_bwd", dt(a), P(a), P(b), P(dy), P(da), P(db), a.numel(), accumulate, S())
 
 
-def colsum(x2d, out, accumulate=False):
+def colsum(x2d, out, accumulate=False, defer=False):
     C = x2d.shape[-1]
     Pn = x2d.numel() // C
+    plan = _WGRAD_PLAN if (defer and GLUE_REDUCE and PROFILE is None and out.is_contiguous()) else None
+    if plan is not None:
+        partial = plan.slab(256 * C * 4)
+        rows = (ctypes.c_int * 1)()
+        _call("dh_colsum_partial", dt(x2d), P(x2d), Pn, C, P(partial), rows, S())
+        plan.add_colsum(partial, rows[0], C, out, accumulate)
+        return
     ws = workspace(1024 * C * 4 + 1024, x2d.device)
     _call("dh_colsum", dt(x2d), P(x2d), Pn, C, P(out), accumulate, P(ws), S())
 
@@ -1573,6 +1708,32 @@
     ws = workspace(4096, logits_nchw.device)
     _call("dh_focal_loss", P(logits_nchw), P(target), B, C, H * W, alpha, grad_scale, P(loss), P(dl), P(ws), S())
     return loss, dl
+
+
+STEP_GLUE = os.environ.get("DAHITRA_STEP_GLUE", "1") != "0"
+GLUE_REDUCE = STEP_GLUE
+GLUE_STEM_COMBINE = STEP_GLUE
+GLUE_TICKET = STEP_GLUE and os.environ.get("DAHITRA_FOCAL_TICKET", "0") == "1"
+
+
+class PackedDlogits:
+
+    def __init__(self, dlp, shape):
+        self.dlp, self.shape, self.device = dlp, tuple(shape), dlp.device
+
+
+def head_dlp_buffer(N, H, W, device):
+    return (torch.zeros(_head_dlp_shape(N, H, W, 2, torch.bfloat16), dtype=torch.int32, device=device),
+            torch.zeros(4, dtype=torch.int32, device=device))
+
+
+def focal_loss_packed(logits_nchw, target, dlp, ticket, grad_scale=1.0, alpha=0.5):
+    B, C, H, W = logits_nchw.shape
+    assert C <= 2 and dlp.dtype == torch.int32 and tuple(dlp.shape) == (B, H + 2, W + 2) and (ticket is None or ticket.dtype == torch.int32)
+    loss = torch.empty((), dtype=torch.float32, device=logits_nchw.device)
+    ws = workspace(4096, logits_nchw.device)
+    _call("dh_focal_loss_packed", P(logits_nchw), P(target), B, C, H, W, alpha, grad_scale, P(loss), P(dlp), P(ws), P(ticket), S())
+    return loss, PackedDlogits(dlp, logits_nchw.shape)
 
 
 def cross_entropy_fwd(logits_nchw, target, ignore_index=255):
diff --git a/include/dahitra_hip.h b/include/dahitra_hip.h
--- a/include/dahitra_hip.h
+++ b/include/dahitra_hip.h
@@ -62,6 +62,10 @@
 int dh_wgrad_batch_end(void* stream);
 int dh_wgrad_batch_abort(void);
 int dh_wgrad_reduce_multi(const void* jobs_dev, int njobs, int total_blocks, void* stream);
+int dh_wgrad_reduce_multi2(const void* jobs_dev, int njobs, int total_blocks, void* stream);
+int dh_wgrad_reduce_job2_size(void);
+int dh_stem_wgrad_bn_partial(const void* xs16, const void* d, const void* y, const float* coef, int groups, int N, int OH, int OW,
+                             float* dw2, int use_tr, void* workspace, int* splitk_out, void* stream);
 int dh_pack_phase_weights(int dtype, const float* w_oihw, const float* bias, int Cin, void* fwd, void* dgrad, float* bias4,
                           void* stream);
 long dh_conv2d_wgrad_phase_workspace_size(int N, int H, int W, int Cin);
@@ -77,6 +81,8 @@
                    int dgrad_inner, void* dgrad, void* stream);
 int dh_pack_weights_multi(const void* jobs_dev, int njobs, int total_blocks, void* stream);
 int dh_pack_job_size(void);
+int dh_step_prologue_multi(const void* jobs_dev, int njobs, int total_blocks, void* stream);
+int dh_step_prologue_job_size(void);
 int dh_zero_insert2(int dtype, const void* dy, void* z, int N, int OH, int OW, int H, int W, int C, void* stream);
 int dh_add_coarse(int dtype, void* x, const void* coarse, int N, int OH, int OW, int H, int W, int C, void* stream);
 
@@ -193,6 +199,7 @@
 int dh_absdiff(int dtype, const void* a, const void* b, void* y, long n, void* stream);
 int dh_absdiff_bwd(int dtype, const void* a, const void* b, const void* dy, void* da, void* db, long n, int accumulate, void* stream);
 int dh_colsum(int dtype, const void* x, long P, int C, float* out, int accumulate, void* workspace, void* stream);
+int dh_colsum_partial(int dtype, const void* x, long P, int C, float* partial, int* rows_out, void* stream);
 int dh_cast_from_f32(int dtype, const float* src, void* dst, long n, void* stream);
 int dh_cast_to_f32(int dtype, const void* src, float* dst, long n, int accumulate, void* stream);
 
@@ -307,6 +314,8 @@
 int dh_focal_loss(const float* logits_nchw, const long long* target, int B, int C, long HW, float alpha,
                   float grad_scale, float* loss_out, float* dlogits_nchw, void* workspace, void* stream);
 int dh_argmax_nchw(const float* logits_nchw, long long* mask, int B, int C, long HW, void* stream);
+int dh_focal_loss_packed(const float* logits_nchw, const long long* target, int B, int C, int H, int W, float alpha,
+                         float grad_scale, float* loss_out, void* dlp, void* workspace, void* ticket, void* stream);
 int dh_cross_entropy_fwd(const float* logits_nchw, const long long* target, int B, int C, long HW, int ignore_index,
                          float* out_dev, void* workspace, void* stream);
 int dh_cross_entropy_bwd(const float* logits_nchw, const long long* target, int B, int C, long HW, int ignore_index,
```

Measured after the change: 9804 image-pairs/s (median of 6 runs). No clear change (+0.6%).
